# jzlianglu/pykaldi2

Measured on AMD Instinct MI355X. Metric: iRTF (hrs audio/hr) 3x512 BLSTM LF-MMI, LibriSpeech-shaped synthetic utterances, higher is better.
Workload: dtype f32 (GEMMs: bf16x3 split, f32 accumulate)

## Files before the change

include/pk2hip.h:

```cpp
#ifndef PK2HIP_H_
#define PK2HIP_H_

#include <stddef.h>
#include <stdint.h>

#ifdef __cplusplus
extern "C" {
#endif

typedef enum {
  PK2_OK = 0,
  PK2_ERR_INVALID = -1,
  PK2_ERR_HIP = -2,
  PK2_ERR_LIMIT = -3,
  PK2_ERR_IO = -4,
  PK2_ERR_NUMERIC = -5
} pk2_status;

const char* pk2_last_error(void);
int pk2_version(void);

typedef struct pk2_den_graph pk2_den_graph;

int pk2_den_graph_create(int32_t num_states, int32_t num_pdfs, int64_t num_arcs,
                         const int32_t* arc_src, const int32_t* arc_dst,
                         const int32_t* arc_pdf, const float* arc_prob,
                         int32_t start_state, pk2_den_graph** out);
int pk2_den_graph_from_openfst(const char* path, int32_t num_pdfs, pk2_den_graph** out);
int pk2_den_graph_destroy(pk2_den_graph* g);
int pk2_den_graph_info(const pk2_den_graph* g, int32_t* num_states, int32_t* num_pdfs,
                       int64_t* num_arcs);
int pk2_den_graph_initial_probs(const pk2_den_graph* g, float* host_out);

int32_t pk2_den_graph_path(const pk2_den_graph* g, int32_t num_seqs);
int32_t pk2_den_graph_persist_form(const pk2_den_graph* g, int32_t num_seqs);
int pk2_den_graph_plan(const pk2_den_graph* g, int32_t num_seqs, int32_t max_frames, int32_t out[8]);

typedef struct {
  const int32_t* arc_src;
  const int32_t* arc_dst;
  const int32_t* arc_pdf;
  const float* arc_weight;
  const int32_t* frame_off;
  const int32_t* state_off;
  const int32_t* final_state;
  const float* final_weight;
  const int32_t* final_off;
  int64_t total_arcs;
  int64_t max_seq_arcs;
} pk2_num_batch;

size_t pk2_chain_workspace_bytes(const pk2_den_graph* g, int32_t num_seqs, int32_t max_frames,
                                 int64_t num_total_states);

int pk2_chain_objf_and_deriv(const pk2_den_graph* g, const float* logits, int64_t seq_stride,
                             int64_t frame_stride, const int32_t* lengths, int32_t num_seqs,
                             const pk2_num_batch* num, float leaky_hmm_coefficient,
                             float xent_regularize, float l2_regularize, float weight,
                             float* grad, int64_t grad_seq_stride, int64_t grad_frame_stride,
                             float* out, void* workspace, size_t workspace_bytes, void* stream);

int pk2_chain_objf_and_deriv_op(const pk2_den_graph* g, const float* logits, int64_t seq_stride,
                                int64_t frame_stride, const int32_t* lengths, int32_t num_seqs,
                                const pk2_num_batch* num, float leaky_hmm_coefficient,
                                float xent_regularize, float l2_regularize, float weight,
                                float* grad, int64_t grad_seq_stride, int64_t grad_frame_stride,
                                float* out, void* workspace, size_t workspace_bytes, float grad_scale,
                                float* objf_sum, void* stream);

int pk2_chain_den_fwd_bwd(const pk2_den_graph* g, const float* logits, int64_t seq_stride,
                          int64_t frame_stride, const int32_t* lengths, int32_t num_seqs,
                          float leaky_hmm_coefficient, float* den_logprob, float* gamma,
                          int64_t gamma_seq_stride, int64_t gamma_frame_stride, void* workspace,
                          size_t workspace_bytes, void* stream);

int pk2_chain_debug_flags(const float* num_lp, const float* den_lp, const float* alpha_beta_product,
                          const int32_t* lengths, int32_t N, float weight, float* out, int32_t* flags, void* stream);

int pk2_chain_debug_num_route(int32_t out[4]);

int pk2_split_to_phones(const int32_t* tid_tstate, const int32_t* tid_phone, const uint8_t* tid_flags,
                        int32_t num_tids, const int32_t* alignment, int32_t T, int32_t* phones,
                        int32_t* durations, int32_t* num_phones, int32_t* ok);

typedef struct pk2_sup_model pk2_sup_model;
pk2_sup_model* pk2_sup_model_create(int32_t max_phone, const int32_t* phone2entry, int32_t num_entries,
                                    const int32_t* entry_state_off, const int32_t* state_fwd_class,
                                    const int32_t* state_loop_class, const int32_t* state_trans_off,
                                    const int32_t* trans_dst, int32_t num_tuples, const int32_t* tuples,
                                    int32_t context_width, int32_t central_position, int32_t num_nodes,
                                    const int32_t* node_kind, const int32_t* node_key, const int32_t* node_a,
                                    const int32_t* node_b, int32_t pool_size, const int32_t* pool);
void pk2_sup_model_destroy(pk2_sup_model* m);
int pk2_sup_model_pdf(const pk2_sup_model* m, const int32_t* window, int32_t pdf_class, int32_t* pdf);

typedef struct pk2_supervision pk2_supervision;
pk2_supervision* pk2_supervision_create(const pk2_sup_model* m, const int32_t* phones,
                                        const int32_t* durations, int32_t num_phones, int32_t subsampling,
                                        int32_t left_tolerance, int32_t right_tolerance);
void pk2_supervision_destroy(pk2_supervision* s);
void pk2_supervision_sizes(const pk2_supervision* s, int32_t* frames, int32_t* num_states, int32_t* num_arcs,
                           int32_t* num_final, int32_t* num_allowed);
int pk2_supervision_copy(const pk2_supervision* s, int32_t* arc_src, int32_t* arc_dst, int32_t* arc_pdf,
                         float* arc_weight, int32_t* frame_off, int32_t* state_time, int32_t* final_state,
                         float* final_weight, int32_t* allowed_off, int32_t* allowed_phones);

typedef struct pk2_lexicon pk2_lexicon;
pk2_lexicon* pk2_lexicon_create(int32_t num_states, int32_t start, int64_t num_arcs, const int32_t* src, const int32_t* dst,
                                const int32_t* ilabel, const int32_t* olabel, const float* weight, const float* final_cost,
                                const int32_t* disambig, int32_t num_disambig);
pk2_lexicon* pk2_lexicon_from_openfst(const char* path, const int32_t* disambig, int32_t num_disambig);
void pk2_lexicon_destroy(pk2_lexicon* lexicon);
typedef struct pk2_align_model pk2_align_model;
pk2_align_model* pk2_align_model_create(const pk2_sup_model* m, int32_t num_tuples, const int32_t* tuples, int32_t num_tids,
                                        const double* log_probs, double transition_scale, double self_loop_scale);
void pk2_align_model_destroy(pk2_align_model* model);
typedef struct pk2_align_graphs pk2_align_graphs;
pk2_align_graphs* pk2_align_compile(const pk2_align_model* model, const pk2_lexicon* lexicon, int32_t num_utts,
                                    const int32_t* word_off, const int32_t* words, const int32_t* frames);
void pk2_align_graphs_destroy(pk2_align_graphs* graphs);
int pk2_align_graphs_info(const pk2_align_graphs* graphs, int32_t utt, int32_t* status, int32_t* num_states, int32_t* num_arcs);
const char* pk2_align_graphs_error(const pk2_align_graphs* graphs, int32_t utt);
int pk2_align_graphs_copy(const pk2_align_graphs* graphs, int32_t utt, int32_t* in_off, int32_t* arc_src, int32_t* arc_tid,
                          int32_t* arc_pdf, float* arc_weight, float* final_cost);
int64_t pk2_align_graphs_packed_words(const pk2_align_graphs* graphs);
int pk2_align_graphs_pack(const pk2_align_graphs* graphs, int32_t* out);
size_t pk2_align_workspace_bytes(const pk2_align_graphs* graphs);
int pk2_align_use_lds(const pk2_align_graphs* graphs);
int pk2_align_viterbi(const pk2_align_graphs* graphs, const int32_t* packed_dev, const float* loglikes, int64_t seq_stride,
                      int64_t frame_stride, int32_t num_pdfs, int32_t Tmax, float acoustic_scale, float beam,
                      int32_t* alignment, float* costs, int32_t* status, void* workspace, size_t workspace_bytes,
                      void* stream);

size_t pk2_num_graph_workspace_bytes(const pk2_align_graphs* graphs);
int pk2_num_graph_use_lds(const pk2_align_graphs* graphs);
int pk2_num_graph_fwd_bwd(const pk2_align_graphs* graphs, const int32_t* packed_dev, const float* logits, int64_t seq_stride,
                          int64_t frame_stride, int32_t num_pdfs, int32_t Tmax, float scale, float* grad, int64_t grad_seq_stride,
                          int64_t grad_frame_stride, float* logprob, int32_t* status, void* workspace, size_t workspace_bytes,
                          void* stream);
size_t pk2_chain_graph_workspace_bytes(const pk2_den_graph* g, const pk2_align_graphs* graphs);
int pk2_chain_objf_and_deriv_graph(const pk2_den_graph* g, const float* logits, int64_t seq_stride, int64_t frame_stride,
                                   const pk2_align_graphs* graphs, const int32_t* packed_dev, float leaky_hmm_coefficient,
                                   float xent_regularize, float l2_regularize, float weight, float* grad,
                                   int64_t grad_seq_stride, int64_t grad_frame_stride, float* out, void* workspace,
                                   size_t workspace_bytes, void* stream);
int pk2_chain_objf_and_deriv_graph_op(const pk2_den_graph* g, const float* logits, int64_t seq_stride, int64_t frame_stride,
                                      const pk2_align_graphs* graphs, const int32_t* packed_dev, float leaky_hmm_coefficient,
                                      float xent_regularize, float l2_regularize, float weight, float* grad,
                                      int64_t grad_seq_stride, int64_t grad_frame_stride, float* out, void* workspace,
                                      size_t workspace_bytes, float grad_scale, float* objf_sum, void* stream);

int pk2_sim_apply_rir(const float* wav, int64_t n, const float* rir, int32_t k, int32_t delay, float* out,
                      void* stream);
int pk2_sim_apply_rir_dev(const float* wav, int64_t n, const float* rir, int32_t k, const int32_t* delay, float* out,
                          void* stream);
int pk2_sim_power(const float* x, int64_t n, double* stats, void* stream);
int pk2_sim_add_noise(float* mixed, int64_t n, const float* noise, int64_t m, int64_t start, float snr_db,
                      const double* sig_stats, const double* noise_stats, void* stream);
int pk2_sim_gain_norm(float* x, int64_t n, const double* stats, void* stream);

#define PK2_SIM_MAX_SEGS 16
typedef struct {
  const float* wav;
  const float* rir;
  float* out;
  float* early;
  const int32_t* delay_dev;
  int64_t n;
  int32_t k;
  int32_t delay;
} pk2_sim_rir_job;
int pk2_sim_apply_rir_mc(const pk2_sim_rir_job* jobs, int32_t njobs, int32_t channels, int32_t early_taps, void* stream);

typedef struct {
  float* x;
  int64_t count;
} pk2_sim_seg;
int pk2_sim_power_seg(const pk2_sim_seg* segs, int32_t nseg, double* stats, void* stream);
int pk2_sim_gain_norm_seg(const pk2_sim_seg* segs, int32_t nseg, const double* stats, double* gain, void* stream);

typedef struct {
  const float* sig;
  const float* sig2;
  float* pos;
  float* pos2;
  int64_t n;
  int64_t start;
  double spr_db;
} pk2_sim_mix_src;
int pk2_sim_mix(const pk2_sim_mix_src* srcs, int32_t nsrc, int32_t channels, int64_t T, const double* stats, float* mixed,
                double* scales, void* stream);
int pk2_sim_add_noise_mc(float* mixed, int64_t n, const float* noise, int64_t m, int32_t channels, int64_t start,
                         float snr_db, int32_t repeat, const double* sig_stats, const double* noise_stats, void* stream);

typedef struct pk2_resample_plan pk2_resample_plan;
#define PK2_RESAMPLE_MAX_TAPS 1024
int pk2_resample_plan_create(int32_t rate_in, int32_t rate_out, double cutoff_hz, int32_t num_zeros,
                             pk2_resample_plan** plan);
int pk2_resample_plan_destroy(pk2_resample_plan* plan);
int pk2_resample_plan_info(const pk2_resample_plan* plan, int32_t* iu, int32_t* ou, int32_t* max_taps, int32_t* tile,
                           int64_t* table_bytes);
int pk2_resample_plan_export(const pk2_resample_plan* plan, int32_t* first, int32_t* taps, float* weights);
int64_t pk2_resample_num_output(const pk2_resample_plan* plan, int64_t n_in);

#define PK2_RESAMPLE_MAX_JOBS 32
typedef struct {
  const pk2_resample_plan* plan;
  const float* in;
  int64_t n_in;
  float* out;
  int64_t n_out;
  float gain;
} pk2_resample_job;
int pk2_resample_batch(const pk2_resample_job* jobs, int32_t njobs, void* stream);
#define PK2_RESAMPLE_PATH_NONE 0
#define PK2_RESAMPLE_PATH_LDS 1
#define PK2_RESAMPLE_PATH_MEM 2
int pk2_resample_last_path(int32_t* path);

int pk2_iso_spectra(const double* tau, const double* g, const float* draws, uint64_t seed, int32_t channels, int32_t points,
                    int32_t bins, float* X, void* stream);
int pk2_iso_gauss(uint64_t seed, int32_t points, int32_t bins, float* out, void* stream);

int pk2_irfft_pow2_f32(const float* X, int32_t rows, int32_t n, float* out, void* stream);

int64_t pk2_stft_num_frames(int64_t n, int32_t frame_len, int32_t frame_shift);
int pk2_stft_f32(const float* const* rows, int32_t R, int64_t n, int32_t fft_size, int32_t frame_len, int32_t frame_shift,
                 const float* window, const float* dither, int32_t use_seed, uint64_t seed, float* out, void* stream);
int pk2_istft_f32(const float* X, int32_t R, int32_t N, int32_t fft_size, int32_t frame_len, int32_t frame_shift,
                  const float* window, float* work, float* out, void* stream);
int pk2_mask_power(const float* spec, int64_t count, float* power, void* stream);
size_t pk2_mask_count_workspace_bytes(int32_t S);
int pk2_mask_count_threshold(const float* power, int32_t S, int64_t m, double energy_threshold, void* work, size_t work_bytes,
                             float* out, void* stream);
int pk2_mask_ibm(const float* clean, const float* distorted, int32_t S, int32_t N, int32_t F, float snr_factor, int32_t soft,
                 const float* thr, const float* vad, float* mask, void* stream);

#define PK2_RIR_F64 16
#define PK2_RIR_I64 12
int32_t pk2_rirgen_segment_samples(void);
int pk2_rirgen(const double* item_f64, const int64_t* item_i64, const double* pos, const int32_t* wg, int32_t nwg,
               const int32_t* row_item, int32_t nrows, int64_t total, void* acc, float* out, int32_t* delay,
               void* stream);

typedef struct pk2_fbank pk2_fbank;
int pk2_fbank_create(const float* mel_80x257, pk2_fbank** out);
int pk2_fbank_destroy(pk2_fbank* fb);
int32_t pk2_fbank_num_frames(int64_t num_samples);
int pk2_fbank_compute(const pk2_fbank* fb, const float* wav, const int64_t* wav_off,
                      int32_t num_utts, float* feats, const int64_t* feat_row_off,
                      int32_t apply_cmn, void* stream);
int pk2_pad_roll_subsample(const float* feats, const int64_t* feat_row_off, int32_t num_utts,
                           int32_t max_t, int32_t shift, int32_t subsample, float* x,
                           int32_t out_t, int32_t time_major, void* stream);

int pk2_mvn_apply(const float* x, const float* mean, const float* stdv, int64_t rows, int32_t dim,
                  float* y, void* stream);

#define PK2_SPEC_MAX_FREQ_MASKS 4
#define PK2_SPEC_MAX_TIME_MASKS 16
#define PK2_SPEC_PLAN_STRIDE (2 + 2 * PK2_SPEC_MAX_FREQ_MASKS + 2 * PK2_SPEC_MAX_TIME_MASKS)
int pk2_spec_augment(const float* in, float* out, const int64_t* row_off , int32_t n,
                     int64_t total_rows, const int32_t* plan , int32_t has_warp,
                     float fill, void* stream);

#define PK2_BF_MAX_CHANNELS 8
#define PK2_BF_MAX_MASKS 4
#define PK2_BF_MAX_UTTS 32
#define PK2_BF_FRAMES_PER_PART 32
#define PK2_BF_REF_SNR (-1)
size_t pk2_bf_workspace_bytes(const int32_t* frames, int32_t B, int32_t C, int32_t F, int32_t K, int32_t complement);
int pk2_bf_cov(const float* const* spec, const float* const* masks, const int32_t* frames, int32_t B, int32_t C, int32_t F,
               int32_t K, int32_t complement, void* work, size_t work_bytes, float* phi, void* stream);
int pk2_bf_mvdr_weights(const float* const* phi_s, const float* const* phi_n, int32_t B, int32_t C, int32_t F, int32_t ref,
                        double diag_load, void* work, size_t work_bytes, float* w, int32_t* ref_index, int32_t* nonfinite,
                        void* stream);
int pk2_bf_apply(const float* const* spec, const float* const* w, const int32_t* frames, int32_t B, int32_t C, int32_t F,
                 float* const* out, void* stream);

#define PK2_WPE_MAX_CHANNELS 8
#define PK2_WPE_MAX_ORDER 80
#define PK2_WPE_MAX_DELAY 8
#define PK2_WPE_MAX_ITERS 8
#define PK2_WPE_MAX_UTTS 32
#define PK2_WPE_FRAMES_PER_PART 1024
size_t pk2_wpe_workspace_bytes(const int32_t* frames, int32_t B, int32_t C, int32_t F, int32_t taps, int32_t delay);
int pk2_wpe_power(const float* const* spec, const int32_t* frames, int32_t B, int32_t C, int32_t F, float* const* power,
                  void* stream);
int pk2_wpe_corr(const float* const* spec, const float* const* weight, const int32_t* frames, int32_t B, int32_t C, int32_t F,
                 int32_t taps, int32_t delay, void* work, size_t work_bytes, float* R, float* P, void* stream);
int pk2_wpe_solve(const float* R, const float* P, int32_t B, int32_t C, int32_t F, int32_t taps, double diag_load, void* work,
                  size_t work_bytes, float* G, int32_t* nonfinite, void* stream);
int pk2_wpe_filter(const float* const* spec, const float* G, const int32_t* frames, int32_t B, int32_t C, int32_t F,
                   int32_t taps, int32_t delay, float* const* out, float* const* power_out, void* stream);
int pk2_wpe(const float* const* spec, const int32_t* frames, int32_t B, int32_t C, int32_t F, int32_t taps, int32_t delay,
            int32_t iters, double diag_load, void* work, size_t work_bytes, float* const* out, int32_t* nonfinite,
            void* stream);

#define PK2_CGMM_MAX_ITERS 32
size_t pk2_cgmm_workspace_bytes(const int32_t* frames, int32_t B, int32_t C, int32_t F, int32_t K);
int pk2_cgmm_init(const float* const* spec, const float* const* init, const float* const* activity, const int32_t* frames,
                  int32_t B, int32_t C, int32_t F, int32_t K, void* work, size_t work_bytes, float* R, float* log_alpha,
                  void* stream);
int pk2_cgmm_factor(const float* R, const float* log_alpha, int32_t B, int32_t C, int32_t F, int32_t K, double diag_load,
                    float* linv, float* bias, int32_t* bad, int32_t* nonfinite, void* stream);
int pk2_cgmm_posteriors(const float* const* spec, const float* const* activity, const int32_t* frames, int32_t B, int32_t C,
                        int32_t F, int32_t K, const float* linv, const float* bias, const int32_t* bad, void* work,
                        size_t work_bytes, float* const* lam, float* const* phi, double* ll, void* stream);
int pk2_cgmm_update(const float* const* spec, const float* const* lam, const float* const* phi, const float* const* activity,
                    const int32_t* frames, int32_t B, int32_t C, int32_t F, int32_t K, void* work, size_t work_bytes, float* R,
                    float* log_alpha, void* stream);
int pk2_cgmm(const float* const* spec, const float* const* init, const float* const* activity, const int32_t* frames, int32_t B,
             int32_t C, int32_t F, int32_t K, int32_t iters, double diag_load, int32_t purity, void* work, size_t work_bytes,
             float* const* masks, float* R, float* log_alpha, double* ll, int32_t* nonfinite, void* stream);

#define PK2_PERM_ALIGN_MAX_REFINE 8
size_t pk2_perm_align_workspace_bytes(const int32_t* frames, int32_t B, int32_t F, int32_t K);
int pk2_perm_align(const float* const* masks, const float* cov, const float* log_alpha, const int32_t* frames, int32_t B,
                   int32_t C, int32_t F, int32_t K, int32_t refine, int32_t noise_last, void* work, size_t work_bytes,
                   float* const* out_masks, float* out_cov, float* out_log_alpha, int32_t* perm, float* margin, void* stream);

int pk2_softmax_ce_fwd_bwd(const float* logits, int64_t row_stride, const int64_t* targets,
                           int64_t ignore_index, int64_t rows, int32_t num_classes,
                           float* loss_sum, int32_t* count, float* grad, int64_t grad_row_stride,
                           float* logprob_out , void* stream);
int pk2_softmax_ce_fwd_bwd_mean(const float* logits, int64_t row_stride, const int64_t* targets,
                                int64_t ignore_index, int64_t rows, int32_t num_classes,
                                float* loss_sum, int32_t* count, float* grad, int64_t grad_row_stride, void* stream);
int pk2_scale_inplace_ratio(float* data, int64_t n, const float* num_dev, const float* den_dev, void* stream);
int pk2_scale_by_count(float* data, int64_t n, float numerator, const int32_t* count_den,
                       void* stream);
int pk2_scale_by_scalars(const float* in, float* out, int64_t n, const float* mul_dev, const int32_t* count_den_dev,
                         void* stream);

int pk2_gemm_f32(int32_t transa, int32_t transb, int32_t M, int32_t N, int32_t K, float alpha,
                 const float* A, int64_t lda, const float* B, int64_t ldb, float beta, float* C,
                 int64_t ldc, const float* bias, void* stream);
int pk2_gemm_f32_act(int32_t transa, int32_t transb, int32_t M, int32_t N, int32_t K, float alpha,
                     const float* A, int64_t lda, const float* B, int64_t ldb, float beta, float* C,
                     int64_t ldc, const float* bias, int32_t act, const float* gate, int64_t ldg, void* stream);
int pk2_gemm_f32_seg(int32_t transa, int32_t transb, int32_t M, int32_t N, int32_t K, int32_t nseg, float alpha,
                     const float* A, int64_t lda, int64_t segA, const float* B, int64_t ldb, int64_t segB, float beta,
                     float* C, int64_t ldc, const float* bias, int32_t act, const float* gate, int64_t ldg,
                     void* stream);
int pk2_gemm_f32_batched(int32_t transa, int32_t transb, int32_t M, int32_t N, int32_t K, float alpha,
                         const float* A, int64_t lda, int64_t strideA0, int64_t strideA1, const float* B,
                         int64_t ldb, int64_t strideB0, int64_t strideB1, float beta, float* C, int64_t ldc,
                         int64_t strideC0, int64_t strideC1, int32_t n0, int32_t n1, void* stream);
int pk2_gemm_set_arith(int32_t arith);
int pk2_gemm_get_arith(void);
int pk2_gemm_f32_tn_colsum(int32_t M, int32_t N, int32_t K, float alpha, const float* A, int64_t lda, const float* B,
                           int64_t ldb, float beta, float* C, int64_t ldc, float* colsum, void* stream);
int pk2_colsum_f32(const float* A, int64_t lda, int32_t M, int32_t N, float beta, float* out,
                   void* stream);

size_t pk2_lstm_fwd_workspace_floats(int32_t B, int32_t H, int32_t num_dirs);
int pk2_lstm_layer_fwd(const float* gx, const float* whh, const float* bhh, int32_t B, int32_t T,
                       int32_t H, int32_t num_dirs, float* y, float* gates, float* cells,
                       void* workspace, void* stream);
int pk2_lstm_layer_fwd_xproj(const float* gx, const float* whh, const float* bhh, int32_t B, int32_t T,
                             int32_t H, int32_t num_dirs, float* y, float* gates, float* cells, void* workspace,
                             const float* inp, int32_t in_size, const float* w_ih, const float* b_ih,
                             int32_t* gx_done, void* stream);
int pk2_lstm_persist_status(uint32_t* abort_flag);
#define PK2_LSTM_PATH_NONE 0
#define PK2_LSTM_PATH_SEQ 1
#define PK2_LSTM_PATH_BIG 2
#define PK2_LSTM_PATH_BIG_AG 3
#define PK2_LSTM_PATH_STEP_SMALL 4
#define PK2_LSTM_PATH_STEP_BIG 5
int pk2_lstm_last_path(int32_t* fwd, int32_t* bwd);
size_t pk2_lstm_bwd_scratch_floats(int32_t B, int32_t H, int32_t num_dirs);
int pk2_lstm_layer_bwd(const float* dy, const float* whh, const float* gates, const float* cells,
                       int32_t B, int32_t T, int32_t H, int32_t num_dirs, float* dgx,
                       float* scratch, void* stream);
int pk2_lstm_layer_bwd_bias(const float* dy, const float* whh, const float* gates, const float* cells,
                            int32_t B, int32_t T, int32_t H, int32_t num_dirs, float* dgx, float* scratch,
                            float* dbias_ih, float* dbias_hh, int32_t* bias_done, void* stream);
size_t pk2_lstm_bwd_wgrad_workspace_floats(int32_t B, int32_t H, int32_t num_dirs);
int pk2_lstm_layer_bwd_wgrad(const float* dy, const float* whh, const float* gates, const float* cells, const float* y,
                             int32_t B, int32_t T, int32_t H, int32_t num_dirs, float* dgx, float* scratch,
                             float* dbias_ih, float* dbias_hh, float* dwhh, float* wgrad_ws, int32_t* bias_done,
                             int32_t* whh_done, void* stream);

int pk2_layernorm_fwd(const float* x, const float* res, const float* gamma, const float* beta, int64_t rows,
                      int32_t C, float eps, float* sum_out, float* y, float* mean, float* rstd, void* stream);
int pk2_layernorm_bwd(const float* dy, const float* s, const float* mean, const float* rstd,
                      const float* gamma, int64_t rows, int32_t C, float* ds, float* dgamma, float* dbeta,
                      void* stream);
int pk2_softmax_mask_fwd(float* scores, const float* src_mask, const uint8_t* key_padding, int32_t B, int32_t H,
                         int32_t T, void* stream);
int pk2_softmax_bwd(const float* P, float* dP, int32_t BH, int32_t T, void* stream);

int pk2_attention_fwd(const float* qkv, int32_t T, int32_t B, int32_t H, int32_t head_dim, float scale,
                      const float* src_mask, const uint8_t* key_padding, float dropout_p, uint64_t seed, float* ctx,
                      float* lse, void* stream);
int pk2_attention_bwd(const float* qkv, const float* ctx, const float* dctx, const float* lse, int32_t T, int32_t B,
                      int32_t H, int32_t head_dim, float scale, const float* src_mask, const uint8_t* key_padding,
                      float dropout_p, uint64_t seed, float* dqkv, float* dsum, void* stream);
int pk2_attention_bwd_part(int32_t parts, const float* qkv, const float* ctx, const float* dctx, const float* lse, int32_t T,
                           int32_t B, int32_t H, int32_t head_dim, float scale, const float* src_mask,
                           const uint8_t* key_padding, float dropout_p, uint64_t seed, float* dqkv, float* dsum, void* stream);
int pk2_relu_fwd(float* x, int64_t n, void* stream);
int pk2_relu_bwd(const float* y, float* dy, int64_t n, void* stream);
int pk2_add_inplace(float* a, const float* b, int64_t n, void* stream);

int pk2_dropout_f32(const float* x, float* y, int64_t n, float p, uint64_t seed, void* stream);

int pk2_grad_norm(const float* grad, int64_t n, float* norm_out, void* workspace,
                  size_t workspace_bytes, void* stream);
size_t pk2_grad_norm_workspace_bytes(int64_t n);
int pk2_adam_step(float* param, const float* grad, float* exp_avg, float* exp_avg_sq,
                  float* max_exp_avg_sq , int64_t n, float lr, float beta1,
                  float beta2, float eps, float weight_decay, int64_t step, float max_norm,
                  const float* norm, float grad_scale, void* stream);
int pk2_sgd_step(float* param, const float* grad, float* momentum_buf ,
                 int64_t n, float lr, float momentum, float weight_decay, int32_t first_step,
                 float max_norm, const float* norm, float grad_scale, void* stream);

int pk2_persist_guard_status(uint32_t* raised);
int pk2_persist_guard_clear(void);
int pk2_persist_guard_raise(void* stream);
int pk2_persist_guard_export(float* slot, void* stream);
int pk2_persist_guard_import(const float* slot, uint32_t stamp, void* stream);
int pk2_persist_guard_verdict(uint32_t stamp, uint32_t* ready, uint32_t* raised);

typedef struct pk2_decode_graph pk2_decode_graph;

int pk2_decode_graph_create(int32_t num_states, int32_t start_state, int64_t num_arcs,
                            const int32_t* arc_src, const int32_t* arc_dst, const int32_t* arc_ilabel,
                            const float* arc_weight, const float* final_cost, pk2_decode_graph** out);
int pk2_decode_graph_from_openfst(const char* path, pk2_decode_graph** out);
int pk2_decode_graph_create_words(int32_t num_states, int32_t start_state, int64_t num_arcs,
                                  const int32_t* arc_src, const int32_t* arc_dst, const int32_t* arc_ilabel,
                                  const int32_t* arc_olabel, const float* arc_weight, const float* final_cost,
                                  pk2_decode_graph** out);
int pk2_decode_graph_link_words(const pk2_decode_graph* g, int64_t num_links, const int32_t* src_state,
                                const int32_t* dst_state, const int32_t* tid, const float* graph_cost,
                                int32_t* word_out);
int pk2_decode_graph_destroy(pk2_decode_graph* g);
int pk2_decode_graph_info(const pk2_decode_graph* g, int32_t* num_states, int64_t* num_arcs,
                          int32_t* max_ilabel);

typedef struct {
  float beam;
  float lattice_beam;
  float beam_delta;
  float acoustic_scale;
  int32_t max_active;
  int32_t min_active;
  int32_t tokens_per_frame;
  int32_t links_per_frame;
} pk2_decoder_opts;

typedef struct pk2_lattice_batch pk2_lattice_batch;
int pk2_lattice_batch_create(const pk2_decode_graph* g, const int32_t* lengths_host, int32_t num_seq,
                             const pk2_decoder_opts* opts, pk2_lattice_batch** out);
size_t pk2_lattice_batch_bytes(const pk2_lattice_batch* b);
int pk2_lattice_batch_destroy(pk2_lattice_batch* b);

int pk2_lattice_decode(pk2_lattice_batch* b, const float* loglikes, int64_t seq_stride,
                       int64_t frame_stride, int32_t num_pdfs, const int32_t* tid2pdf, int32_t num_tids,
                       void* workspace, void* stream);
int pk2_lattice_persist_status(int32_t* state, uint32_t* abort_flag);
int pk2_lattice_summary(const pk2_lattice_batch* b, const void* workspace, int32_t* status,
                        int32_t* num_tokens, int32_t* num_links, float* best_cost, void* stream);
int pk2_lattice_fb_rerun(const pk2_lattice_batch* b, void* workspace, int32_t* rerun, void* stream);
int pk2_lattice_mmi(const pk2_lattice_batch* b, void* workspace, const int32_t* ref_tids,
                    int64_t ref_stride, const int32_t* tid2pdf, double lm_scale, double acoustic_scale,
                    int32_t drop_frames, float* post, int64_t post_seq_stride,
                    int64_t post_frame_stride, double* lat_like, void* stream);
int pk2_lattice_mpe(const pk2_lattice_batch* b, void* workspace, const int32_t* ref_tids,
                    int64_t ref_stride, const int32_t* tid2pdf, const int32_t* tid2phone,
                    const uint8_t* phone_is_silence, int32_t criterion, int32_t one_silence_class,
                    double lm_scale, double acoustic_scale, float* post, int64_t post_seq_stride,
                    int64_t post_frame_stride, double* score, void* stream);
size_t pk2_lattice_nbest_bytes(const pk2_lattice_batch* b, int32_t num_paths, int64_t total_tokens, int64_t total_links,
                               int32_t distinct, int32_t label_cap);
int pk2_lattice_nbest(const pk2_lattice_batch* b, void* workspace, void* scratch, int64_t total_tokens,
                      int64_t total_links, int32_t num_paths, int32_t distinct, int32_t label_mode,
                      const int32_t* tid2label, int32_t num_tids, double lm_scale, double acoustic_scale,
                      int32_t label_cap, int32_t* num_hyp, int32_t* hyp_path, float* path_cost, int32_t* path_nlab,
                      int32_t* path_labels, int32_t* path_tids, void* stream);
int pk2_lattice_mwe(const pk2_lattice_batch* b, void* workspace, void* scratch, int64_t total_tokens,
                    int64_t total_links, int32_t num_paths, int32_t distinct, int32_t label_mode,
                    const int32_t* tid2label, int32_t num_tids, double lm_scale, double acoustic_scale,
                    int32_t label_cap, int32_t equal_weight, const int32_t* sup, int64_t sup_stride,
                    const int32_t* sup_len, const int32_t* tid2pdf, int32_t num_pdfs, float* grad,
                    int64_t grad_seq_stride, int64_t grad_frame_stride, double* loss, void* stream);
int pk2_lattice_rescore(const pk2_lattice_batch* b, void* workspace, const float* loglikes, int64_t seq_stride,
                        int64_t frame_stride, int32_t num_pdfs, const int32_t* tid2pdf, int32_t num_tids,
                        float old_acoustic_scale, void* stream);
int pk2_lattice_posteriors(const pk2_lattice_batch* b, void* workspace, const int32_t* tid2pdf, double lm_scale,
                           double acoustic_scale, float post_sign, float* post, int64_t post_seq_stride,
                           int64_t post_frame_stride, double* lat_like, void* stream);
int pk2_lattice_ts(const pk2_lattice_batch* b, void* workspace, const float* loglikes_S, int64_t seq_stride,
                   int64_t frame_stride, int32_t num_pdfs, const int32_t* tid2pdf, int32_t num_tids,
                   float old_acoustic_scale, double lm_scale, double acoustic_scale, float* grad,
                   int64_t grad_seq_stride, int64_t grad_frame_stride, double* loss, double* like_T, double* like_S,
                   void* stream);
int pk2_lattice_export(const pk2_lattice_batch* b, const void* workspace, int32_t n, int32_t* num_tokens,
                       int32_t* num_links, int32_t* tok_frame, int32_t* tok_state, float* tok_cost,
                       float* tok_final, int32_t* link_src, int32_t* link_dst, int32_t* link_tid,
                       float* link_graph, float* link_ac, void* stream);

typedef struct pk2_det_lattice pk2_det_lattice;
int pk2_lattice_determinize(int32_t num_states, int32_t start, int64_t num_arcs, const int32_t* src, const int32_t* dst,
                            const int32_t* word, const int32_t* tid, const float* graph, const float* acoustic,
                            const float* final_cost, double beam, int64_t max_states, pk2_det_lattice** out);
int pk2_det_lattice_sizes(const pk2_det_lattice* h, int32_t* num_states, int32_t* start, int64_t* num_arcs,
                          int64_t* arc_tids, int64_t* final_tids);
int pk2_det_lattice_export(const pk2_det_lattice* h, int32_t* src, int32_t* dst, int32_t* word, float* graph,
                           float* acoustic, int64_t* tid_off, int32_t* tids, float* final_graph, float* final_acoustic,
                           int64_t* final_tid_off, int32_t* final_tids);
void pk2_det_lattice_destroy(pk2_det_lattice* h);

typedef struct pk2_comm pk2_comm;
int32_t pk2_comm_unique_id_bytes(void);
int pk2_comm_unique_id(void* id_out);
int pk2_comm_init(int32_t rank, int32_t world, const void* unique_id, pk2_comm** out);
int pk2_allreduce_bucket(pk2_comm* comm, float* buf, int64_t count, void* stream);
int pk2_allreduce_guarded(pk2_comm* comm, float* buf, int64_t count, float* guard_slot, void* stream);
int pk2_comm_info(const pk2_comm* comm, int32_t* rank, int32_t* world, char* lib_path, int32_t lib_path_bytes);
int pk2_comm_destroy(pk2_comm* comm);

int pk2_stream_create_cu_mask(int32_t cus_per_xcd, void** stream_out);
int pk2_stream_destroy(void* stream);
int pk2_debug_where(int32_t* out, int32_t blocks, void* stream);
int pk2_debug_peer_reduce(float* dst, const float* src, int64_t n, int32_t blocks, int32_t passes, void* stream);

#ifdef __cplusplus
}
#endif
#endif
```

pykaldi2_amd/_lib.py:

```python
import ctypes as C
import os

import torch

_HERE = os.path.dirname(os.path.abspath(__file__))
LIB_PATH = os.environ.get("PK2_LIB") or os.path.join(_HERE, "libpk2hip.so")


class Pk2Error(RuntimeError):
    pass


class NumBatch(C.Structure):
    _fields_ = [("arc_src", C.c_void_p), ("arc_dst", C.c_void_p), ("arc_pdf", C.c_void_p),
                ("arc_weight", C.c_void_p), ("frame_off", C.c_void_p), ("state_off", C.c_void_p),
                ("final_state", C.c_void_p), ("final_weight", C.c_void_p), ("final_off", C.c_void_p),
                ("total_arcs", C.c_int64), ("max_seq_arcs", C.c_int64)]


class DecoderOpts(C.Structure):
    _fields_ = [("beam", C.c_float), ("lattice_beam", C.c_float), ("beam_delta", C.c_float),
                ("acoustic_scale", C.c_float), ("max_active", C.c_int32), ("min_active", C.c_int32),
                ("tokens_per_frame", C.c_int32), ("links_per_frame", C.c_int32)]


class SimRirJob(C.Structure):
    _fields_ = [("wav", C.c_void_p), ("rir", C.c_void_p), ("out", C.c_void_p), ("early", C.c_void_p),
                ("delay_dev", C.c_void_p), ("n", C.c_int64), ("k", C.c_int32), ("delay", C.c_int32)]


class SimSeg(C.Structure):
    _fields_ = [("x", C.c_void_p), ("count", C.c_int64)]


class SimMixSrc(C.Structure):
    _fields_ = [("sig", C.c_void_p), ("sig2", C.c_void_p), ("pos", C.c_void_p), ("pos2", C.c_void_p),
                ("n", C.c_int64), ("start", C.c_int64), ("spr_db", C.c_double)]


class ResampleJob(C.Structure):
    _fields_ = [("plan", C.c_void_p), ("inp", C.c_void_p), ("n_in", C.c_int64), ("out", C.c_void_p), ("n_out", C.c_int64),
                ("gain", C.c_float)]


SIM_MAX_SEGS = 16
RESAMPLE_MAX_JOBS = 32
SPEC_MAX_FREQ_MASKS = 4
SPEC_MAX_TIME_MASKS = 16
SPEC_PLAN_STRIDE = 2 + 2 * SPEC_MAX_FREQ_MASKS + 2 * SPEC_MAX_TIME_MASKS
BF_MAX_CHANNELS = 8
BF_MAX_MASKS = 4
BF_FRAMES_PER_PART = 32
BF_REF_SNR = -1
CGMM_MAX_ITERS = 32
PERM_ALIGN_MAX_REFINE = 8
WPE_MAX_CHANNELS = 8
WPE_MAX_ORDER = 80
WPE_MAX_DELAY = 8
WPE_MAX_ITERS = 8
WPE_FRAMES_PER_PART = 1024

_vp, _i32, _i64, _f32, _sz = C.c_void_p, C.c_int32, C.c_int64, C.c_float, C.c_size_t

SIGNATURES = {
    "pk2_last_error": (C.c_char_p, []),
    "pk2_version": (C.c_int, []),
    "pk2_den_graph_create": (C.c_int, [_i32, _i32, _i64, _vp, _vp, _vp, _vp, _i32, C.POINTER(_vp)]),
    "pk2_den_graph_from_openfst": (C.c_int, [C.c_char_p, _i32, C.POINTER(_vp)]),
    "pk2_den_graph_destroy": (C.c_int, [_vp]),
    "pk2_den_graph_info": (C.c_int, [_vp, C.POINTER(_i32), C.POINTER(_i32), C.POINTER(_i64)]),
    "pk2_den_graph_initial_probs": (C.c_int, [_vp, _vp]),
    "pk2_den_graph_arcs_per_lane": (_i32, []),
    "pk2_den_graph_path": (_i32, [_vp, _i32]),
    "pk2_den_graph_persist_form": (_i32, [_vp, _i32]),
    "pk2_den_graph_plan": (C.c_int, [_vp, _i32, _i32, _vp]),
    "pk2_den_graph_debug_ordering": (C.c_int, [_vp, C.c_int, C.POINTER(_i64), C.POINTER(_i32), _vp, _vp,
                                               _vp, _vp, _vp, _vp]),
    "pk2_den_graph_debug_virtual": (C.c_int, [_vp, C.c_int, C.POINTER(_i32), _vp, _vp, _vp, _vp, _vp,
                                              C.POINTER(_i64), _vp, _vp, _vp, C.POINTER(_i32), _vp, _vp]),
    "pk2_den_graph_debug_persist2": (C.c_int, [_vp, C.c_int] + [_vp] * 18),
    "pk2_den_graph_debug_persist2_table": (C.c_int, [_vp, C.c_int, _vp, _vp, _vp, _vp]),
    "pk2_chain_workspace_bytes": (_sz, [_vp, _i32, _i32, _i64]),
    "pk2_chain_objf_and_deriv": (C.c_int, [_vp, _vp, _i64, _i64, _vp, _i32, C.POINTER(NumBatch), _f32,
                                           _f32, _f32, _f32, _vp, _i64, _i64, _vp, _vp, _sz, _vp]),
    "pk2_chain_objf_and_deriv_op": (C.c_int, [_vp, _vp, _i64, _i64, _vp, _i32, C.POINTER(NumBatch), _f32,
                                              _f32, _f32, _f32, _vp, _i64, _i64, _vp, _vp, _sz, _f32, _vp, _vp]),
    "pk2_chain_den_fwd_bwd": (C.c_int, [_vp, _vp, _i64, _i64, _vp, _i32, _f32, _vp, _vp, _i64, _i64,
                                        _vp, _sz, _vp]),
    "pk2_chain_debug_flags": (C.c_int, [_vp, _vp, _vp, _vp, _i32, _f32, _vp, _vp, _vp]),
    "pk2_chain_debug_num_route": (C.c_int, [_vp]),
    "pk2_split_to_phones": (C.c_int, [_vp, _vp, _vp, _i32, _vp, _i32, _vp, _vp, C.POINTER(_i32), C.POINTER(_i32)]),
    "pk2_sup_model_create": (_vp, [_i32, _vp, _i32, _vp, _vp, _vp, _vp, _vp, _i32, _vp, _i32, _i32, _i32, _vp, _vp,
                                   _vp, _vp, _i32, _vp]),
    "pk2_sup_model_destroy": (None, [_vp]),
    "pk2_sup_model_pdf": (C.c_int, [_vp, _vp, _i32, C.POINTER(_i32)]),
    "pk2_supervision_create": (_vp, [_vp, _vp, _vp, _i32, _i32, _i32, _i32]),
    "pk2_supervision_destroy": (None, [_vp]),
    "pk2_supervision_sizes": (None, [_vp, C.POINTER(_i32), C.POINTER(_i32), C.POINTER(_i32), C.POINTER(_i32),
                                     C.POINTER(_i32)]),
    "pk2_supervision_copy": (C.c_int, [_vp, _vp, _vp, _vp, _vp, _vp, _vp, _vp, _vp, _vp, _vp]),
    "pk2_lexicon_create": (_vp, [_i32, _i32, _i64, _vp, _vp, _vp, _vp, _vp, _vp, _vp, _i32]),
    "pk2_lexicon_from_openfst": (_vp, [C.c_char_p, _vp, _i32]),
    "pk2_lexicon_destroy": (None, [_vp]),
    "pk2_align_model_create": (_vp, [_vp, _i32, _vp, _i32, _vp, C.c_double, C.c_double]),
    "pk2_align_model_destroy": (None, [_vp]),
    "pk2_align_compile": (_vp, [_vp, _vp, _i32, _vp, _vp, _vp]),
    "pk2_align_graphs_destroy": (None, [_vp]),
    "pk2_align_graphs_info": (C.c_int, [_vp, _i32, C.POINTER(_i32), C.POINTER(_i32), C.POINTER(_i32)]),
    "pk2_align_graphs_error": (C.c_char_p, [_vp, _i32]),
    "pk2_align_graphs_copy": (C.c_int, [_vp, _i32, _vp, _vp, _vp, _vp, _vp, _vp]),
    "pk2_align_graphs_packed_words": (_i64, [_vp]),
    "pk2_align_graphs_pack": (C.c_int, [_vp, _vp]),
    "pk2_align_workspace_bytes": (_sz, [_vp]),
    "pk2_align_use_lds": (C.c_int, [_vp]),
    "pk2_align_viterbi": (C.c_int, [_vp, _vp, _vp, _i64, _i64, _i32, _i32, _f32, _f32, _vp, _vp, _vp, _vp, _sz, _vp]),
    "pk2_num_graph_workspace_bytes": (_sz, [_vp]),
    "pk2_num_graph_use_lds": (C.c_int, [_vp]),
    "pk2_num_graph_fwd_bwd": (C.c_int, [_vp, _vp, _vp, _i64, _i64, _i32, _i32, _f32, _vp, _i64, _i64, _vp, _vp, _vp, _sz, _vp]),
    "pk2_chain_graph_workspace_bytes": (_sz, [_vp, _vp]),
    "pk2_chain_objf_and_deriv_graph": (C.c_int, [_vp, _vp, _i64, _i64, _vp, _vp, _f32, _f32, _f32, _f32, _vp, _i64, _i64, _vp,
                                                 _vp, _sz, _vp]),
    "pk2_chain_objf_and_deriv_graph_op": (C.c_int, [_vp, _vp, _i64, _i64, _vp, _vp, _f32, _f32, _f32, _f32, _vp, _i64, _i64,
                                                    _vp, _vp, _sz, _f32, _vp, _vp]),
    "pk2_decode_graph_create": (C.c_int, [_i32, _i32, _i64, _vp, _vp, _vp, _vp, _vp, C.POINTER(_vp)]),
    "pk2_decode_graph_create_words": (C.c_int, [_i32, _i32, _i64, _vp, _vp, _vp, _vp, _vp, _vp, C.POINTER(_vp)]),
    "pk2_decode_graph_link_words": (C.c_int, [_vp, _i64, _vp, _vp, _vp, _vp, _vp]),
    "pk2_decode_graph_from_openfst": (C.c_int, [C.c_char_p, C.POINTER(_vp)]),
    "pk2_decode_graph_destroy": (C.c_int, [_vp]),
    "pk2_decode_graph_info": (C.c_int, [_vp, C.POINTER(_i32), C.POINTER(_i64), C.POINTER(_i32)]),
    "pk2_lattice_batch_create": (C.c_int, [_vp, _vp, _i32, C.POINTER(DecoderOpts), C.POINTER(_vp)]),
    "pk2_lattice_batch_bytes": (_sz, [_vp]),
    "pk2_lattice_batch_destroy": (C.c_int, [_vp]),
    "pk2_lattice_decode": (C.c_int, [_vp, _vp, _i64, _i64, _i32, _vp, _i32, _vp, _vp]),
    "pk2_lattice_summary": (C.c_int, [_vp, _vp, _vp, _vp, _vp, _vp, _vp]),
    "pk2_lattice_persist_status": (C.c_int, [C.POINTER(C.c_int32), C.POINTER(C.c_uint32)]),
    "pk2_lattice_mmi": (C.c_int, [_vp, _vp, _vp, _i64, _vp, C.c_double, C.c_double, _i32, _vp, _i64, _i64, _vp, _vp]),
    "pk2_lattice_mpe": (C.c_int, [_vp, _vp, _vp, _i64, _vp, _vp, _vp, _i32, _i32, C.c_double, C.c_double, _vp, _i64, _i64,
                                  _vp, _vp]),
    "pk2_lattice_nbest_bytes": (_sz, [_vp, _i32, _i64, _i64, _i32, _i32]),
    "pk2_lattice_nbest": (C.c_int, [_vp, _vp, _vp, _i64, _i64, _i32, _i32, _i32, _vp, _i32, C.c_double, C.c_double, _i32,
                                    _vp, _vp, _vp, _vp, _vp, _vp, _vp]),
    "pk2_lattice_mwe": (C.c_int, [_vp, _vp, _vp, _i64, _i64, _i32, _i32, _i32, _vp, _i32, C.c_double, C.c_double, _i32, _i32,
                                  _vp, _i64, _vp, _vp, _i32, _vp, _i64, _i64, _vp, _vp]),
    "pk2_lattice_rescore": (C.c_int, [_vp, _vp, _vp, _i64, _i64, _i32, _vp, _i32, _f32, _vp]),
    "pk2_lattice_fb_rerun": (C.c_int, [_vp, _vp, _vp, _vp]),
    "pk2_lattice_posteriors": (C.c_int, [_vp, _vp, _vp, C.c_double, C.c_double, _f32, _vp, _i64, _i64, _vp, _vp]),
    "pk2_lattice_ts": (C.c_int, [_vp, _vp, _vp, _i64, _i64, _i32, _vp, _i32, _f32, C.c_double, C.c_double, _vp, _i64, _i64,
                                 _vp, _vp, _vp, _vp]),
    "pk2_lattice_export": (C.c_int, [_vp, _vp, _i32, C.POINTER(_i32), C.POINTER(_i32), _vp, _vp, _vp, _vp, _vp,
                                     _vp, _vp, _vp, _vp, _vp]),
    "pk2_comm_unique_id_bytes": (_i32, []),
    "pk2_comm_unique_id": (C.c_int, [_vp]),
    "pk2_comm_init": (C.c_int, [_i32, _i32, _vp, C.POINTER(_vp)]),
    "pk2_allreduce_bucket": (C.c_int, [_vp, _vp, _i64, _vp]),
    "pk2_allreduce_guarded": (C.c_int, [_vp, _vp, _i64, _vp, _vp]),
    "pk2_comm_info": (C.c_int, [_vp, C.POINTER(_i32), C.POINTER(_i32), C.c_char_p, _i32]),
    "pk2_comm_destroy": (C.c_int, [_vp]),
    "pk2_sim_apply_rir": (C.c_int, [_vp, _i64, _vp, _i32, _i32, _vp, _vp]),
    "pk2_sim_apply_rir_dev": (C.c_int, [_vp, _i64, _vp, _i32, _vp, _vp, _vp]),
    "pk2_sim_power": (C.c_int, [_vp, _i64, _vp, _vp]),
    "pk2_rirgen_segment_samples": (_i32, []),
    "pk2_rirgen": (C.c_int, [_vp, _vp, _vp, _vp, _i32, _vp, _i32, _i64, _vp, _vp, _vp, _vp]),
    "pk2_sim_add_noise": (C.c_int, [_vp, _i64, _vp, _i64, _i64, _f32, _vp, _vp, _vp]),
    "pk2_sim_gain_norm": (C.c_int, [_vp, _i64, _vp, _vp]),
    "pk2_sim_apply_rir_mc": (C.c_int, [C.POINTER(SimRirJob), _i32, _i32, _i32, _vp]),
    "pk2_sim_power_seg": (C.c_int, [C.POINTER(SimSeg), _i32, _vp, _vp]),
    "pk2_sim_gain_norm_seg": (C.c_int, [C.POINTER(SimSeg), _i32, _vp, _vp, _vp]),
    "pk2_sim_mix": (C.c_int, [C.POINTER(SimMixSrc), _i32, _i32, _i64, _vp, _vp, _vp, _vp]),
    "pk2_sim_add_noise_mc": (C.c_int, [_vp, _i64, _vp, _i64, _i32, _i64, _f32, _i32, _vp, _vp, _vp]),
    "pk2_resample_plan_create": (C.c_int, [_i32, _i32, C.c_double, _i32, C.POINTER(_vp)]),
    "pk2_resample_plan_destroy": (C.c_int, [_vp]),
    "pk2_resample_plan_info": (C.c_int, [_vp, C.POINTER(_i32), C.POINTER(_i32), C.POINTER(_i32), C.POINTER(_i32),
                                         C.POINTER(_i64)]),
    "pk2_resample_plan_export": (C.c_int, [_vp, _vp, _vp, _vp]),
    "pk2_resample_num_output": (_i64, [_vp, _i64]),
    "pk2_resample_batch": (C.c_int, [C.POINTER(ResampleJob), _i32, _vp]),
    "pk2_resample_last_path": (C.c_int, [C.POINTER(_i32)]),
    "pk2_iso_spectra": (C.c_int, [_vp, _vp, _vp, C.c_uint64, _i32, _i32, _i32, _vp, _vp]),
    "pk2_iso_gauss": (C.c_int, [C.c_uint64, _i32, _i32, _vp, _vp]),
    "pk2_irfft_pow2_f32": (C.c_int, [_vp, _i32, _i32, _vp, _vp]),
    "pk2_stft_num_frames": (_i64, [_i64, _i32, _i32]),
    "pk2_stft_f32": (C.c_int, [C.POINTER(_vp), _i32, _i64, _i32, _i32, _i32, _vp, _vp, _i32, C.c_uint64, _vp, _vp]),
    "pk2_istft_f32": (C.c_int, [_vp, _i32, _i32, _i32, _i32, _i32, _vp, _vp, _vp, _vp]),
    "pk2_mask_power": (C.c_int, [_vp, _i64, _vp, _vp]),
    "pk2_mask_count_workspace_bytes": (_sz, [_i32]),
    "pk2_mask_count_threshold": (C.c_int, [_vp, _i32, _i64, C.c_double, _vp, _sz, _vp, _vp]),
    "pk2_mask_ibm": (C.c_int, [_vp, _vp, _i32, _i32, _i32, _f32, _i32, _vp, _vp, _vp, _vp]),
    "pk2_fbank_create": (C.c_int, [_vp, C.POINTER(_vp)]),
    "pk2_fbank_destroy": (C.c_int, [_vp]),
    "pk2_fbank_num_frames": (_i32, [_i64]),
    "pk2_fbank_compute": (C.c_int, [_vp, _vp, _vp, _i32, _vp, _vp, _i32, _vp]),
    "pk2_pad_roll_subsample": (C.c_int, [_vp, _vp, _i32, _i32, _i32, _i32, _vp, _i32, _i32, _vp]),
    "pk2_mvn_apply": (C.c_int, [_vp, _vp, _vp, _i64, _i32, _vp, _vp]),
    "pk2_spec_augment": (C.c_int, [_vp, _vp, _vp, _i32, _i64, _vp, _i32, _f32, _vp]),
    "pk2_bf_workspace_bytes": (_sz, [_vp, _i32, _i32, _i32, _i32, _i32]),
    "pk2_bf_cov": (C.c_int, [C.POINTER(_vp), C.POINTER(_vp), C.POINTER(_i32), _i32, _i32, _i32, _i32, _i32, _vp, _sz, _vp, _vp]),
    "pk2_bf_mvdr_weights": (C.c_int, [C.POINTER(_vp), C.POINTER(_vp), _i32, _i32, _i32, _i32, C.c_double, _vp, _sz, _vp, _vp,
                                      _vp, _vp]),
    "pk2_bf_apply": (C.c_int, [C.POINTER(_vp), C.POINTER(_vp), C.POINTER(_i32), _i32, _i32, _i32, C.POINTER(_vp), _vp]),
    "pk2_wpe_workspace_bytes": (_sz, [_vp, _i32, _i32, _i32, _i32, _i32]),
    "pk2_wpe_power": (C.c_int, [C.POINTER(_vp), C.POINTER(_i32), _i32, _i32, _i32, C.POINTER(_vp), _vp]),
    "pk2_wpe_corr": (C.c_int, [C.POINTER(_vp), C.POINTER(_vp), C.POINTER(_i32), _i32, _i32, _i32, _i32, _i32, _vp, _sz, _vp, _vp,
                               _vp]),
    "pk2_wpe_solve": (C.c_int, [_vp, _vp, _i32, _i32, _i32, _i32, C.c_double, _vp, _sz, _vp, _vp, _vp]),
    "pk2_wpe_filter": (C.c_int, [C.POINTER(_vp), _vp, C.POINTER(_i32), _i32, _i32, _i32, _i32, _i32, C.POINTER(_vp),
                                 C.POINTER(_vp), _vp]),
    "pk2_wpe": (C.c_int, [C.POINTER(_vp), C.POINTER(_i32), _i32, _i32, _i32, _i32, _i32, _i32, C.c_double, _vp, _sz,
                          C.POINTER(_vp), _vp, _vp]),
    "pk2_cgmm_workspace_bytes": (_sz, [_vp, _i32, _i32, _i32, _i32]),
    "pk2_cgmm_init": (C.c_int, [C.POINTER(_vp), C.POINTER(_vp), C.POINTER(_vp), C.POINTER(_i32), _i32, _i32, _i32, _i32, _vp, _sz,
                                _vp, _vp, _vp]),
    "pk2_cgmm_factor": (C.c_int, [_vp, _vp, _i32, _i32, _i32, _i32, C.c_double, _vp, _vp, _vp, _vp, _vp]),
    "pk2_cgmm_posteriors": (C.c_int, [C.POINTER(_vp), C.POINTER(_vp), C.POINTER(_i32), _i32, _i32, _i32, _i32, _vp, _vp, _vp, _vp,
                                      _sz, C.POINTER(_vp), C.POINTER(_vp), _vp, _vp]),
    "pk2_cgmm_update": (C.c_int, [C.POINTER(_vp), C.POINTER(_vp), C.POINTER(_vp), C.POINTER(_vp), C.POINTER(_i32), _i32, _i32,
                                  _i32, _i32, _vp, _sz, _vp, _vp, _vp]),
    "pk2_cgmm": (C.c_int, [C.POINTER(_vp), C.POINTER(_vp), C.POINTER(_vp), C.POINTER(_i32), _i32, _i32, _i32, _i32, _i32,
                           C.c_double, _i32, _vp, _sz, C.POINTER(_vp), _vp, _vp, _vp, _vp, _vp]),
    "pk2_perm_align_workspace_bytes": (_sz, [_vp, _i32, _i32, _i32]),
    "pk2_perm_align": (C.c_int, [C.POINTER(_vp), _vp, _vp, C.POINTER(_i32), _i32, _i32, _i32, _i32, _i32, _i32, _vp, _sz,
                                 C.POINTER(_vp), _vp, _vp, _vp, _vp, _vp]),
    "pk2_softmax_ce_fwd_bwd": (C.c_int, [_vp, _i64, _vp, _i64, _i64, _i32, _vp, _vp, _vp, _i64, _vp, _vp]),
    "pk2_softmax_ce_fwd_bwd_mean": (C.c_int, [_vp, _i64, _vp, _i64, _i64, _i32, _vp, _vp, _vp, _i64, _vp]),
    "pk2_scale_inplace_ratio": (C.c_int, [_vp, _i64, _vp, _vp, _vp]),
    "pk2_scale_by_count": (C.c_int, [_vp, _i64, _f32, _vp, _vp]),
    "pk2_scale_by_scalars": (C.c_int, [_vp, _vp, _i64, _vp, _vp, _vp]),
    "pk2_gemm_f32": (C.c_int, [_i32, _i32, _i32, _i32, _i32, _f32, _vp, _i64, _vp, _i64, _f32, _vp, _i64,
                               _vp, _vp]),
    "pk2_gemm_f32_act": (C.c_int, [_i32, _i32, _i32, _i32, _i32, _f32, _vp, _i64, _vp, _i64, _f32, _vp, _i64, _vp, _i32, _vp, _i64,
                                   _vp]),
    "pk2_gemm_f32_seg": (C.c_int, [_i32, _i32, _i32, _i32, _i32, _i32, _f32, _vp, _i64, _i64, _vp, _i64, _i64, _f32, _vp, _i64, _vp,
                                   _i32, _vp, _i64, _vp]),
    "pk2_gemm_f32_batched": (C.c_int, [_i32, _i32, _i32, _i32, _i32, _f32, _vp, _i64, _i64, _i64, _vp, _i64, _i64, _i64,
                                       _f32, _vp, _i64, _i64, _i64, _i32, _i32, _vp]),
    "pk2_gemm_f32_tn_colsum": (C.c_int, [_i32, _i32, _i32, _f32, _vp, _i64, _vp, _i64, _f32, _vp, _i64, _vp, _vp]),
    "pk2_gemm_set_arith": (C.c_int, [_i32]),
    "pk2_gemm_get_arith": (C.c_int, []),
    "pk2_layernorm_fwd": (C.c_int, [_vp, _vp, _vp, _vp, _i64, _i32, _f32, _vp, _vp, _vp, _vp, _vp]),
    "pk2_layernorm_bwd": (C.c_int, [_vp, _vp, _vp, _vp, _vp, _i64, _i32, _vp, _vp, _vp, _vp]),
    "pk2_softmax_mask_fwd": (C.c_int, [_vp, _vp, _vp, _i32, _i32, _i32, _vp]),
    "pk2_softmax_bwd": (C.c_int, [_vp, _vp, _i32, _i32, _vp]),
    "pk2_attention_fwd": (C.c_int, [_vp, _i32, _i32, _i32, _i32, _f32, _vp, _vp, _f32, C.c_uint64, _vp, _vp, _vp]),
    "pk2_attention_bwd": (C.c_int, [_vp, _vp, _vp, _vp, _i32, _i32, _i32, _i32, _f32, _vp, _vp, _f32, C.c_uint64, _vp,
                                    _vp, _vp]),
    "pk2_attention_bwd_part": (C.c_int, [_i32, _vp, _vp, _vp, _vp, _i32, _i32, _i32, _i32, _f32, _vp, _vp, _f32, C.c_uint64,
                                         _vp, _vp, _vp]),
    "pk2_relu_fwd": (C.c_int, [_vp, _i64, _vp]),
    "pk2_relu_bwd": (C.c_int, [_vp, _vp, _i64, _vp]),
    "pk2_add_inplace": (C.c_int, [_vp, _vp, _i64, _vp]),
    "pk2_colsum_f32": (C.c_int, [_vp, _i64, _i32, _i32, _f32, _vp, _vp]),
    "pk2_lstm_fwd_workspace_floats": (_sz, [_i32, _i32, _i32]),
    "pk2_lstm_layer_fwd": (C.c_int, [_vp, _vp, _vp, _i32, _i32, _i32, _i32, _vp, _vp, _vp, _vp, _vp]),
    "pk2_lstm_layer_fwd_xproj": (C.c_int, [_vp, _vp, _vp, _i32, _i32, _i32, _i32, _vp, _vp, _vp, _vp, _vp, _i32, _vp, _vp,
                                           C.POINTER(_i32), _vp]),
    "pk2_lstm_persist_status": (C.c_int, [C.POINTER(C.c_uint32)]),
    "pk2_lstm_last_path": (C.c_int, [C.POINTER(_i32), C.POINTER(_i32)]),
    "pk2_lattice_determinize": (C.c_int, [_i32, _i32, _i64, _vp, _vp, _vp, _vp, _vp, _vp, _vp, C.c_double, _i64, C.POINTER(_vp)]),
    "pk2_det_lattice_sizes": (C.c_int, [_vp, C.POINTER(_i32), C.POINTER(_i32), C.POINTER(_i64), C.POINTER(_i64), C.POINTER(_i64)]),
    "pk2_det_lattice_export": (C.c_int, [_vp] * 12),
    "pk2_det_lattice_destroy": (None, [_vp]),
    "pk2_persist_guard_status": (C.c_int, [C.POINTER(C.c_uint32)]),
    "pk2_persist_guard_clear": (C.c_int, []),
    "pk2_persist_guard_raise": (C.c_int, [_vp]),
    "pk2_persist_guard_export": (C.c_int, [_vp, _vp]),
    "pk2_persist_guard_import": (C.c_int, [_vp, C.c_uint32, _vp]),
    "pk2_persist_guard_verdict": (C.c_int, [C.c_uint32, C.POINTER(C.c_uint32), C.POINTER(C.c_uint32)]),
    "pk2_lstm_bwd_scratch_floats": (_sz, [_i32, _i32, _i32]),
    "pk2_lstm_layer_bwd_bias": (C.c_int, [_vp, _vp, _vp, _vp, _i32, _i32, _i32, _i32, _vp, _vp, _vp, _vp, C.POINTER(_i32), _vp]),
    "pk2_lstm_layer_bwd": (C.c_int, [_vp, _vp, _vp, _vp, _i32, _i32, _i32, _i32, _vp, _vp, _vp]),
    "pk2_lstm_bwd_wgrad_workspace_floats": (_sz, [_i32, _i32, _i32]),
    "pk2_lstm_layer_bwd_wgrad": (C.c_int, [_vp, _vp, _vp, _vp, _vp, _i32, _i32, _i32, _i32, _vp, _vp, _vp, _vp, _vp, _vp,
                                           C.POINTER(_i32), C.POINTER(_i32), _vp]),
    "pk2_dropout_f32": (C.c_int, [_vp, _vp, _i64, _f32, C.c_uint64, _vp]),
    "pk2_grad_norm": (C.c_int, [_vp, _i64, _vp, _vp, _sz, _vp]),
    "pk2_grad_norm_workspace_bytes": (_sz, [_i64]),
    "pk2_adam_step": (C.c_int, [_vp, _vp, _vp, _vp, _vp, _i64, _f32, _f32, _f32, _f32, _f32, _i64, _f32,
                                _vp, _f32, _vp]),
    "pk2_sgd_step": (C.c_int, [_vp, _vp, _vp, _i64, _f32, _f32, _f32, _i32, _f32, _vp, _f32, _vp]),
    "pk2_stream_create_cu_mask": (C.c_int, [_i32, C.POINTER(_vp)]),
    "pk2_stream_destroy": (C.c_int, [_vp]),
    "pk2_debug_where": (C.c_int, [_vp, _i32, _vp]),
    "pk2_debug_peer_reduce": (C.c_int, [_vp, _vp, _i64, _i32, _i32, _vp]),
}

_lib = None


def lib():
    global _lib
    if _lib is None:
        if not os.path.exists(LIB_PATH):
            raise Pk2Error("%s is missing: run `python -c 'import __graft_entry__ as g; g.build()'` "
                           "(hipcc --offload-arch=gfx950).  There is no CPU fallback." % LIB_PATH)
        handle = C.CDLL(LIB_PATH)
        for name, (res, args) in SIGNATURES.items():
            fn = getattr(handle, name)
            fn.restype = res
            fn.argtypes = args
        _lib = handle
    return _lib


def h2d(host, device):
    import numpy as np
    t = torch.from_numpy(host) if isinstance(host, np.ndarray) else host
    if torch.device(device).type != "cuda" or t.is_cuda or t.numel() == 0:
        return t.to(device)
    return t.contiguous().pin_memory().to(device, non_blocking=True)


def check(status):
    if status != 0:
        msg = lib().pk2_last_error()
        raise Pk2Error("libpk2hip status %d: %s" % (status, msg.decode() if msg else ""))


def persist_guard_raised():
    flag = C.c_uint32(0)
    check(lib().pk2_persist_guard_status(C.byref(flag)))
    return flag.value != 0


def check_persist_guard(where, raised=None):
    if persist_guard_raised() if raised is None else raised:
        raise Pk2Error("%s: a persistent kernel (one-launch LSTM recurrence / denominator / lattice decoder) timed out on "
                       "this device; its output was poisoned with NaN and the optimiser kernels have been leaving the "
                       "weights untouched since.  Typical causes: the GPU is shared with another process, or fewer than "
                       "256 CUs are available to the launch.  PK2_LSTM_SEQ=0 PK2_LSTM_BIG_PERSIST=0 PK2_DEN_PERSIST=0 "
                       "PK2_LAT_DECODER=frames select the launch-per-step kernels." % where)


def ptr(t):
    if t is None:
        return None
    if isinstance(t, torch.Tensor):
        return C.c_void_p(t.data_ptr())
    return C.c_void_p(t.ctypes.data)


def stream_ptr(device=None):
    return C.c_void_p(torch.cuda.current_stream(device).cuda_stream)


def require_gpu():
    if not torch.cuda.is_available():
        raise Pk2Error("pykaldi2_amd needs an MI355X (torch.cuda.is_available() is False); "
                       "there is no CPU fallback")
```

pykaldi2_amd/csrc/gemm_bf16x3.h:

```cpp
#pragma once
#include "gemm_tile.h"

namespace pk2 {

typedef __bf16 bf16x8_t __attribute__((ext_vector_type(8)));
typedef unsigned int u32x4_t __attribute__((ext_vector_type(4)));

template <int TILES> struct GeoX {
  static constexpr int BMN = 64 * TILES;
  static constexpr int BK = TILES == 2 ? 16 : 32;
  static constexpr int NKG = BK / 8;
  static constexpr int NQ = BMN / 4;
  static constexpr int SW = NQ + 4;
  template <bool KC> static constexpr int sp() { return KC ? BMN + 4 : NQ + 3 * SW; }
  template <bool KC> static constexpr int slots() { return 3 * NKG * sp<KC>(); }
  template <bool KC> __device__ static __forceinline__ int slot(int row) { return KC ? row : (row >> 2) + SW * (row & 3); }
};

__device__ __forceinline__ unsigned pk_bf16(float a, float b) {
  typedef __bf16 bf16x2_t __attribute__((ext_vector_type(2)));
  typedef float f32x2_t __attribute__((ext_vector_type(2)));
  f32x2_t v = {a, b};
  bf16x2_t r = __builtin_convertvector(v, bf16x2_t);
  return __builtin_bit_cast(unsigned, r);
}
__device__ __forceinline__ void split_pair(float x0, float x1, unsigned& h, unsigned& m, unsigned& l) {
  h = pk_bf16(x0, x1);
#ifdef PK2_X3_DBG_NOSPLIT
  m = h; l = h; return;
#endif
  const float r0 = x0 - __uint_as_float(h << 16), r1 = x1 - __uint_as_float(h & 0xffff0000u);
  m = pk_bf16(r0, r1);
  const float s0 = r0 - __uint_as_float(m << 16), s1 = r1 - __uint_as_float(m & 0xffff0000u);
  l = pk_bf16(s0, s1);
}

template <bool KC, int TILES> struct PieceMap {
  int row[2], k[2];
  int kg, d;
  __device__ __forceinline__ PieceMap() {
    const int t = threadIdx.x;
    if (KC) {
      if (TILES == 2) { row[0] = t >> 2; row[1] = (t >> 2) + 64; k[0] = k[1] = (t & 3) * 4; }
      else            { row[0] = row[1] = t >> 2; k[0] = (t & 3) * 4; k[1] = k[0] + 16; }
      kg = d = 0;
    } else {
      const int q = (t & 7) + 8 * ((t >> 5) & (TILES == 2 ? 3 : 1));
      d = (t >> 3) & 3;
      kg = TILES == 2 ? (t >> 7) : (t >> 6);
      row[0] = row[1] = 4 * q;
      k[0] = 8 * kg + 2 * d;
      k[1] = k[0] + 1;
    }
  }
};

template <bool KC, int TILES>
__device__ __forceinline__ void xslab_pointers(const PieceMap<KC, TILES>& pm, const float* __restrict__ base, int64_t ld, int r0,
                                               int k0, int R, const float* (&ptr)[2], int64_t* step) {
#pragma unroll
  for (int h = 0; h < 2; ++h) {
    if (KC) ptr[h] = base + (int64_t)min(r0 + pm.row[h], R - 1) * ld + k0 + pm.k[h];
    else    ptr[h] = base + (int64_t)(k0 + pm.k[h]) * ld + min(r0 + pm.row[h], R - 4);
  }
  *step = KC ? (int64_t)GeoX<TILES>::BK : (int64_t)GeoX<TILES>::BK * ld;
}

template <bool KC, int TILES>
__device__ __forceinline__ void xload_general(const PieceMap<KC, TILES>& pm, const float* __restrict__ base, int64_t ld, int r0,
                                              int k0, int R, int K, bool vec, float4 (&reg)[2]) {
#pragma unroll
  for (int h = 0; h < 2; ++h) {
    const int gr = r0 + pm.row[h], gk = k0 + pm.k[h];
    float4 v = make_float4(0.f, 0.f, 0.f, 0.f);
    if (KC) {
      if (gr < R) {
        const float* p = base + (int64_t)gr * ld + gk;
        if (vec && gk + 3 < K) v = *reinterpret_cast<const float4*>(p);
        else {
          if (gk + 0 < K) v.x = p[0];
          if (gk + 1 < K) v.y = p[1];
          if (gk + 2 < K) v.z = p[2];
          if (gk + 3 < K) v.w = p[3];
        }
      }
    } else {
      if (gk < K) {
        const float* p = base + (int64_t)gk * ld + gr;
        if (vec && gr + 3 < R) v = *reinterpret_cast<const float4*>(p);
        else {
          if (gr + 0 < R) v.x = p[0];
          if (gr + 1 < R) v.y = p[1];
          if (gr + 2 < R) v.z = p[2];
          if (gr + 3 < R) v.w = p[3];
        }
      }
    }
    reg[h] = v;
  }
}

template <bool KC, int TILES, bool CS = false>
__device__ __forceinline__ void xstore(const PieceMap<KC, TILES>& pm, u32x4_t* __restrict__ tile, const float4 (&reg)[2],
                                       float* cs = nullptr, float csw = 0.f) {
  typedef GeoX<TILES> G;
  constexpr int SP = G::template sp<KC>(), PL = G::NKG * SP;
  if (KC) {
#pragma unroll
    for (int h = 0; h < 2; ++h) {
      unsigned h0, m0, l0, h1, m1, l1;
      split_pair(reg[h].x, reg[h].y, h0, m0, l0);
      split_pair(reg[h].z, reg[h].w, h1, m1, l1);
      const int kq = pm.k[h] >> 2;
      uint2* p = reinterpret_cast<uint2*>(tile + (kq >> 1) * SP + pm.row[h]) + (kq & 1);
      p[0] = make_uint2(h0, h1);
      p[2 * PL] = make_uint2(m0, m1);
      p[4 * PL] = make_uint2(l0, l1);
    }
  } else {
    const float a[4] = {reg[0].x, reg[0].y, reg[0].z, reg[0].w};
    const float b[4] = {reg[1].x, reg[1].y, reg[1].z, reg[1].w};
    unsigned* p = reinterpret_cast<unsigned*>(tile + pm.kg * SP + (pm.row[0] >> 2)) + pm.d;
#pragma unroll
    for (int i = 0; i < 4; ++i) {
      unsigned hh, mm, ll;
      split_pair(a[i], b[i], hh, mm, ll);
      p[4 * (G::SW * i)] = hh;
      p[4 * (G::SW * i + PL)] = mm;
      p[4 * (G::SW * i + 2 * PL)] = ll;
      if (CS) cs[i] = fmaf(csw, a[i] + b[i], cs[i]);
    }
  }
}

template <bool KCA, bool KCB, int TILES>
__device__ __forceinline__ void tile_mainloop_bf16x3(const float* __restrict__ A, int64_t lda, const float* __restrict__ B, int64_t ldb,
                                                     int m0, int n0, int kbeg, int K, int M, int N, bool vecA, bool vecB,
                                                     u32x4_t (*As)[GeoX<TILES>::template slots<KCA>()],
                                                     u32x4_t (*Bs)[GeoX<TILES>::template slots<KCB>()],
                                                     f32x16 (&acc)[TILES][TILES], float* __restrict__ colsum = nullptr,
                                                     bool zero_acc = true) {
  typedef GeoX<TILES> G;
  constexpr int BM = G::BMN, BN = G::BMN, XBK = G::BK, NKG = G::NKG;
  constexpr int SPA = G::template sp<KCA>(), SPB = G::template sp<KCB>();
  const int lane = threadIdx.x & 63, w = threadIdx.x >> 6;
  const int wm = (w >> 1) * 32 * TILES, wn = (w & 1) * 32 * TILES;
  if (zero_acc) {
#pragma unroll
    for (int i = 0; i < TILES; ++i)
#pragma unroll
      for (int j = 0; j < TILES; ++j)
#pragma unroll
        for (int r = 0; r < 16; ++r) acc[i][j][r] = 0.f;
  }
  const int kq = lane >> 5, li = lane & 31;
#ifndef PK2_GEMMX_DEPTH
#define PK2_GEMMX_DEPTH 2
#endif
  constexpr int DEPTH = PK2_GEMMX_DEPTH;
  static_assert(DEPTH % 2 == 0, "an even number of register stages (the LDS buffer is the stage's parity)");
  float4 ra[DEPTH][2], rb[DEPTH][2];
  const PieceMap<KCA, TILES> pma;
  const PieceMap<KCB, TILES> pmb;
  float cs[4] = {0.f, 0.f, 0.f, 0.f};
  const bool do_cs = !KCA && colsum != nullptr;
  auto store_a = [&](u32x4_t* tile, const float4 (&reg)[2], bool real = true) {
    if constexpr (!KCA) { if (do_cs) { xstore<KCA, TILES, true>(pma, tile, reg, cs, real ? 1.f : 0.f); return; } }
    xstore<KCA, TILES>(pma, tile, reg);
  };
  const int nk = (K - kbeg + XBK - 1) / XBK;
  const bool interior = vecA && vecB && (m0 + BM <= M || KCA || ((M & 3) == 0 && M >= 4)) &&
                        (n0 + BN <= N || KCB || ((N & 3) == 0 && N >= 4));
  const float* pa[2]; const float* pb[2];
  int64_t stepA = 0, stepB = 0;
  xslab_pointers<KCA, TILES>(pma, A, lda, m0, kbeg, M, pa, &stepA);
  xslab_pointers<KCB, TILES>(pmb, B, ldb, n0, kbeg, N, pb, &stepB);
  int sa[TILES], sb[TILES];
#pragma unroll
  for (int i = 0; i < TILES; ++i) sa[i] = kq * SPA + G::template slot<KCA>(wm + i * 32 + li);
#pragma unroll
  for (int j = 0; j < TILES; ++j) sb[j] = kq * SPB + G::template slot<KCB>(wn + j * 32 + li);
  auto multiply = [&](auto C_) {
    constexpr int cur = decltype(C_)::value;
#pragma unroll
    for (int s = 0; s < NKG / 2; ++s) {
      bf16x8_t a[3][TILES], b[3][TILES];
#pragma unroll
      for (int p = 0; p < 3; ++p) {
#pragma unroll
        for (int i = 0; i < TILES; ++i) a[p][i] = __builtin_bit_cast(bf16x8_t, As[cur][(p * NKG + 2 * s) * SPA + sa[i]]);
#pragma unroll
        for (int j = 0; j < TILES; ++j) b[p][j] = __builtin_bit_cast(bf16x8_t, Bs[cur][(p * NKG + 2 * s) * SPB + sb[j]]);
      }
#define PK2_X3(PA, PB)                                                                                   \
  _Pragma("unroll") for (int i = 0; i < TILES; ++i) _Pragma("unroll") for (int j = 0; j < TILES; ++j)    \
      acc[i][j] = __builtin_amdgcn_mfma_f32_32x32x16_bf16(a[PA][i], b[PB][j], acc[i][j], 0, 0, 0)
#ifdef PK2_X3_DBG_ONEMFMA
      PK2_X3(0, 0);
      asm volatile("" :: "v"(a[1][0]), "v"(a[2][0]), "v"(b[1][0]), "v"(b[2][0]));
#else
      PK2_X3(2, 0); PK2_X3(0, 2); PK2_X3(1, 1); PK2_X3(1, 0); PK2_X3(0, 1); PK2_X3(0, 0);
#endif
#undef PK2_X3
    }
  };
  auto pipeline = [&](int n, auto fetch) {
    if (n <= 0) return;
#pragma unroll
    for (int i = 0; i < DEPTH; ++i) fetch(min(i, n - 1), ra[i], rb[i]);
    store_a(As[0], ra[0]);
    xstore<KCB, TILES>(pmb, Bs[0], rb[0]);
    lds_barrier();
    fetch(min(DEPTH, n - 1), ra[0], rb[0]);
#ifndef PK2_GEMMX_PIN
#define PK2_GEMMX_PIN 1
#endif
    auto pin = [] { if (PK2_GEMMX_PIN) __builtin_amdgcn_sched_barrier(0); };
    auto slab_step = [&](int kt, auto P) {
      constexpr int st = decltype(P)::value, cur = st & 1, nxt = 1 - cur, sn = (st + 1) % DEPTH;
      multiply(std::integral_constant<int, cur>());
      if (kt + 1 < n) {
        store_a(As[nxt], ra[sn]);
        xstore<KCB, TILES>(pmb, Bs[nxt], rb[sn]);
      }
      lds_barrier();
      if (kt + 1 + DEPTH < n) fetch(kt + 1 + DEPTH, ra[sn], rb[sn]);
    };
    auto steady_step = [&](int kt, auto P) {
      constexpr int st = decltype(P)::value, cur = st & 1, nxt = 1 - cur, sn = (st + 1) % DEPTH;
      multiply(std::integral_constant<int, cur>());
      store_a(As[nxt], ra[sn], kt + 1 < n);
      xstore<KCB, TILES>(pmb, Bs[nxt], rb[sn]);
      lds_barrier();
      fetch(min(kt + 1 + DEPTH, n - 1), ra[sn], rb[sn]);
      pin();
    };
    int kt = 0;
    for (; kt + DEPTH <= n; kt += DEPTH)
      static_for<0, DEPTH>([&](auto S) { steady_step(kt + decltype(S)::value, S); });
    if (kt < n)
      static_for<0, DEPTH>([&](auto S) { if (kt + decltype(S)::value < n) slab_step(kt + decltype(S)::value, S); });
  };
  if (interior) {
    const int nk_fast = (K - kbeg) / XBK;
    pipeline(nk_fast, [&](int ks, float4 (&xa)[2], float4 (&xb)[2]) {
#ifdef PK2_X3_DBG_NOLOAD
      ks = 0;
#endif
#pragma unroll
      for (int h = 0; h < 2; ++h) xa[h] = *reinterpret_cast<const float4*>(pa[h] + ks * stepA);
#pragma unroll
      for (int h = 0; h < 2; ++h) xb[h] = *reinterpret_cast<const float4*>(pb[h] + ks * stepB);
    });
    if (nk > nk_fast) {
      xload_general<KCA, TILES>(pma, A, lda, m0, kbeg + nk_fast * XBK, M, K, vecA, ra[0]);
      xload_general<KCB, TILES>(pmb, B, ldb, n0, kbeg + nk_fast * XBK, N, K, vecB, rb[0]);
      store_a(As[0], ra[0]);
      xstore<KCB, TILES>(pmb, Bs[0], rb[0]);
      lds_barrier();
      multiply(std::integral_constant<int, 0>());
      lds_barrier();
    }
  } else {
    pipeline(nk, [&](int ks, float4 (&xa)[2], float4 (&xb)[2]) {
      xload_general<KCA, TILES>(pma, A, lda, m0, kbeg + ks * XBK, M, K, vecA, xa);
      xload_general<KCB, TILES>(pmb, B, ldb, n0, kbeg + ks * XBK, N, K, vecB, xb);
    });
  }
  if constexpr (!KCA) {
    if (do_cs) {
      float* red = reinterpret_cast<float*>(&As[0][0]);
      for (int r = threadIdx.x; r < BM; r += kGemmThreads) red[r] = 0.f;
      lds_barrier();
#pragma unroll
      for (int i = 0; i < 4; ++i) atomicAdd(&red[pma.row[0] + i], cs[i]);
      lds_barrier();
      for (int r = threadIdx.x; r < BM; r += kGemmThreads)
        if (m0 + r < M) atomicAdd(colsum + m0 + r, red[r]);
      lds_barrier();
    }
  }
}



}
```

pykaldi2_amd/csrc/gemm_f32.hip:

```cpp
#include <algorithm>
#include <cstdlib>
#include <type_traits>

#include "common.h"
#include "gemm_tile.h"
#include "gemm_bf16x3.h"

namespace pk2 {

struct GemmBatch { int n1; int64_t sA0, sA1, sB0, sB1, sC0, sC1; int ksplit, klen; float* colsum = nullptr;
                   int act = 0; const float* gate = nullptr; int64_t ldg = 0;
                   int nseg = 1; int64_t segA = 0, segB = 0; };

#ifndef PK2_GEMMX_WAVES
#define PK2_GEMMX_WAVES 2
#endif
template <int TILES>
__device__ __forceinline__ void gemm_store(const f32x16 (&acc)[TILES][TILES], int M, int N, float alpha, float beta, float* __restrict__ C,
                                           int64_t ldc, const float* __restrict__ bias, int m0, int n0, int wm, int wn, bool atomic,
                                           int act = 0, const float* __restrict__ gate = nullptr, int64_t ldg = 0) {
  const int lane = threadIdx.x & 63;
  const int col_l = lane & 31, row_h = 4 * (lane >> 5);
#pragma unroll
  for (int i = 0; i < TILES; ++i) {
#pragma unroll
    for (int j = 0; j < TILES; ++j) {
      const int gc = n0 + wn + j * 32 + col_l;
      if (gc >= N) continue;
      if (atomic) {
#pragma unroll
        for (int r = 0; r < 16; ++r) {
          const int gr = m0 + wm + i * 32 + (r & 3) + 8 * (r >> 2) + row_h;
          if (gr < M) atomicAdd(C + (int64_t)gr * ldc + gc, alpha * acc[i][j][r]);
        }
        continue;
      }
      const float bv = bias ? bias[gc] : 0.f;
#pragma unroll
      for (int r = 0; r < 16; ++r) {
        const int gr = m0 + wm + i * 32 + (r & 3) + 8 * (r >> 2) + row_h;
        if (gr < M) {
          float* o = C + (int64_t)gr * ldc + gc;
          float v = alpha * acc[i][j][r] + bv;
          if (beta != 0.f) v += beta * (*o);
          if (act == 1) v = fmaxf(v, 0.f);
          else if (act == 2) v = gate[(int64_t)gr * ldg + gc] > 0.f ? v : 0.f;
          *o = v;
        }
      }
    }
  }
}

template <bool TA, bool TB, int TILES, bool X3>
constexpr size_t gemm_smem_bytes() {
  if (X3) return 2 * 16 * (size_t)(GeoX<TILES>::template slots<!TA>() + GeoX<TILES>::template slots<TB>());
  return 2 * sizeof(float) * BK * (size_t)(Geo<TILES>::template ld<!TA>() + Geo<TILES>::template ld<TB>());
}

template <bool TA, bool TB, int TILES, bool X3, bool SEG = false>
__device__ __forceinline__ void gemm_block(void* smem, int M, int N, int K, int kbeg, float alpha, const float* __restrict__ A, int64_t lda,
                                           const float* __restrict__ B, int64_t ldb, float beta, float* __restrict__ C,
                                           int64_t ldc, const float* __restrict__ bias, bool vecA, bool vecB, int m0, int n0,
                                           bool atomic, float* colsum = nullptr, int act = 0, const float* __restrict__ gate = nullptr,
                                           int64_t ldg = 0, int nseg = 1, int64_t segA = 0, int64_t segB = 0) {
  const int tid = threadIdx.x, lane = tid & 63, w = tid >> 6;
  const int wm = (w >> 1) * 32 * TILES, wn = (w & 1) * 32 * TILES;

  f32x16 acc[TILES][TILES];
#ifdef PK2_GEMM_PROFILE
  const long long gp_t0 = wall_clock64();
#endif
  if constexpr (X3) {
    typedef u32x4_t (*StA)[GeoX<TILES>::template slots<!TA>()];
    typedef u32x4_t (*StB)[GeoX<TILES>::template slots<TB>()];
    StA Ax = reinterpret_cast<StA>(smem);
    StB Bx = reinterpret_cast<StB>(reinterpret_cast<u32x4_t*>(smem) + 2 * GeoX<TILES>::template slots<!TA>());
    if constexpr (!SEG) tile_mainloop_bf16x3<!TA, TB, TILES>(A, lda, B, ldb, m0, n0, kbeg, K, M, N, vecA, vecB, Ax, Bx, acc, n0 == 0 ? colsum : nullptr);
    else
      for (int sg = 0; sg < nseg; ++sg)
        tile_mainloop_bf16x3<!TA, TB, TILES>(A + sg * segA, lda, B + sg * segB, ldb, m0, n0, kbeg, K, M, N, vecA, vecB, Ax, Bx, acc, nullptr, sg == 0);
  } else {
    constexpr int LDA = Geo<TILES>::template ld<!TA>(), LDB = Geo<TILES>::template ld<TB>();
    typedef float (*StA)[BK * LDA];
    typedef float (*StB)[BK * LDB];
    StA As = reinterpret_cast<StA>(smem);
    StB Bs = reinterpret_cast<StB>(reinterpret_cast<float*>(smem) + 2 * BK * LDA);
    if constexpr (!SEG) tile_mainloop<!TA, TB, TILES>(A, lda, B, ldb, m0, n0, kbeg, K, M, N, vecA, vecB, As, Bs, acc);
    else
      for (int sg = 0; sg < nseg; ++sg)
        tile_mainloop<!TA, TB, TILES>(A + sg * segA, lda, B + sg * segB, ldb, m0, n0, kbeg, K, M, N, vecA, vecB, As, Bs, acc, sg == 0);
  }
#ifdef PK2_GEMM_PROFILE
  const long long gp_t1 = wall_clock64();
#endif
  gemm_store<TILES>(acc, M, N, alpha, beta, C, ldc, bias, m0, n0, wm, wn, atomic, act, gate, ldg);
#ifdef PK2_GEMM_PROFILE
  asm volatile("s_waitcnt vmcnt(0)" ::: "memory");
#ifndef PK2_GEMM_PROFILE_N
#define PK2_GEMM_PROFILE_N 4096
#define PK2_GEMM_PROFILE_K 1024
#define PK2_GEMM_PROFILE_EVERY 97
#endif
  if (tid == 0 && K == PK2_GEMM_PROFILE_K && N == PK2_GEMM_PROFILE_N && (blockIdx.x + blockIdx.y * gridDim.x) % PK2_GEMM_PROFILE_EVERY == 0) {
    unsigned xcc;
    asm volatile("s_getreg_b32 %0, hwreg(HW_REG_XCC_ID)" : "=s"(xcc));
    printf("gemm tile (%d,%d) of grid (%d,%d) tiles=%d xcc %u: start %lld main loop %lld epilogue %lld (10 ns ticks)\n", blockIdx.x, blockIdx.y,
           gridDim.x, gridDim.y, TILES, xcc & 7u, gp_t0, gp_t1 - gp_t0, wall_clock64() - gp_t1);
  }
#endif
}

template <bool TA, bool TB, int TILES, bool X3, bool SEG = false>
__global__ void __launch_bounds__(kGemmThreads, X3 ? PK2_GEMMX_WAVES : 3) gemm_f32_kernel(int M, int N, int K, float alpha,
                                                                const float* __restrict__ A, int64_t lda,
                                                                const float* __restrict__ B, int64_t ldb,
                                                                float beta, float* __restrict__ C, int64_t ldc,
                                                                const float* __restrict__ bias, bool vecA,
                                                                bool vecB, GemmBatch bt) {
  int kbeg = 0;
  {
    int z = blockIdx.z;
    if (bt.ksplit > 1) {
      kbeg = (z % bt.ksplit) * bt.klen;
      z /= bt.ksplit;
      K = min(K, kbeg + bt.klen);
    }
    const int i0 = z / bt.n1, i1 = z % bt.n1;
    A += i0 * bt.sA0 + i1 * bt.sA1;
    B += i0 * bt.sB0 + i1 * bt.sB1;
    C += i0 * bt.sC0 + i1 * bt.sC1;
  }
  __shared__ __attribute__((aligned(16))) char smem[gemm_smem_bytes<TA, TB, TILES, X3>()];
  gemm_block<TA, TB, TILES, X3, SEG>(smem, M, N, K, kbeg, alpha, A, lda, B, ldb, beta, C, ldc, bias, vecA, vecB,
                                blockIdx.y * Geo<TILES>::BMN, blockIdx.x * Geo<TILES>::BMN, bt.ksplit > 1, bt.colsum, bt.act, bt.gate,
                                bt.ldg, bt.nseg, bt.segA, bt.segB);
}

template <bool TA, bool TB, bool X3>
__global__ void __launch_bounds__(kGemmThreads, X3 ? PK2_GEMMX_WAVES : 3) gemm_f32_bands_kernel(int M, int N, int K, float alpha,
                                                                         const float* __restrict__ A, int64_t lda,
                                                                         const float* __restrict__ B, int64_t ldb,
                                                                         float beta, float* __restrict__ C, int64_t ldc,
                                                                         const float* __restrict__ bias, bool vecA,
                                                                         bool vecB, int nbig, int big_cols, int m_split,
                                                                         int small_cols) {
  const int b = blockIdx.x;
  __shared__ __attribute__((aligned(16))) char smem[std::max(gemm_smem_bytes<TA, TB, 2, X3>(), gemm_smem_bytes<TA, TB, 1, X3>())];
  if (b < nbig) {
    gemm_block<TA, TB, 2, X3>(smem, M, N, K, 0, alpha, A, lda, B, ldb, beta, C, ldc, bias, vecA, vecB, (b / big_cols) * 128,
                              (b % big_cols) * 128, false);
  } else {
    const int s = b - nbig;
    gemm_block<TA, TB, 1, X3>(smem, M, N, K, 0, alpha, A, lda, B, ldb, beta, C, ldc, bias, vecA, vecB, m_split + (s / small_cols) * 64,
                              (s % small_cols) * 64, false);
  }
}

__global__ void __launch_bounds__(256) gemm_prescale_kernel(int M, int N, float beta, float* __restrict__ C,
                                                            int64_t ldc, const float* __restrict__ bias, GemmBatch bt) {
  C += (blockIdx.z / bt.n1) * bt.sC0 + (blockIdx.z % bt.n1) * bt.sC1;
  const int n = blockIdx.x * 256 + threadIdx.x;
  if (n >= N) return;
  const float bv = bias ? bias[n] : 0.f;
  for (int m = blockIdx.y; m < M; m += gridDim.y) {
    float* o = C + (int64_t)m * ldc + n;
    *o = beta == 0.f ? bv : beta * (*o) + bv;
  }
}

__global__ void __launch_bounds__(256) colsum_kernel(const float* __restrict__ A, int64_t lda, int M, int N,
                                                     int rows_per_block, float* __restrict__ out) {
  __shared__ float red[4][64];
  const int n = blockIdx.x * 64 + (threadIdx.x & 63);
  const int part = threadIdx.x >> 6;
  const int m0 = blockIdx.y * rows_per_block, m1 = min(M, m0 + rows_per_block);
  float acc = 0.f;
  if (n < N)
    for (int m = m0 + part; m < m1; m += 4) acc += A[(int64_t)m * lda + n];
  red[part][threadIdx.x & 63] = acc;
  __syncthreads();
  if (part == 0 && n < N)
    atomicAdd(out + n, (red[0][threadIdx.x] + red[1][threadIdx.x]) + (red[2][threadIdx.x] + red[3][threadIdx.x]));
}

__global__ void scale_vec_kernel(float* v, int n, float beta) {
  const int i = blockIdx.x * blockDim.x + threadIdx.x;
  if (i < n) v[i] = beta == 0.f ? 0.f : beta * v[i];
}

}

using namespace pk2;

#ifndef PK2_GEMM_ARITH_DEFAULT
#define PK2_GEMM_ARITH_DEFAULT 1
#endif
extern "C" int pk2_colsum_f32(const float* A, int64_t lda, int32_t M, int32_t N, float beta, float* out, void* stream_);
static int g_gemm_arith = -1;
static int gemm_arith() {
  if (g_gemm_arith < 0) {
    const char* e = getenv("PK2_GEMM_ARITH");
    g_gemm_arith = e ? (strcmp(e, "f32") == 0 ? 0 : 1) : PK2_GEMM_ARITH_DEFAULT;
  }
  return g_gemm_arith;
}
extern "C" int pk2_gemm_set_arith(int32_t arith) {
  PK2_REQUIRE(arith == 0 || arith == 1, "gemm_set_arith: 0 = f32, 1 = bf16x3");
  g_gemm_arith = arith;
  return PK2_OK;
}
extern "C" int pk2_gemm_get_arith(void) { return gemm_arith(); }

#ifndef PK2_GEMM_MIN_KSLICE
#define PK2_GEMM_MIN_KSLICE 256
#endif
static int gemm_launch(int transa, int transb, int M, int N, int K, float alpha, const float* A, int64_t lda,
                       const float* B, int64_t ldb, float beta, float* C, int64_t ldc, const float* bias,
                       int n0, const GemmBatch& bt_in, bool aligned_strides, hipStream_t stream) {
  GemmBatch bt = bt_in;
  const bool x3 = gemm_arith() == 1;
  const bool vecA = aligned_strides && (reinterpret_cast<uintptr_t>(A) & 15) == 0 && (lda & 3) == 0;
  const bool vecB = aligned_strides && (reinterpret_cast<uintptr_t>(B) & 15) == 0 && (ldb & 3) == 0;
  const int64_t big_tiles = (int64_t)((N + 127) / 128) * ((M + 127) / 128) * n0 * bt.n1;
  const char* force = getenv("PK2_GEMM_TILES");
  int tiles = force ? atoi(force) : ((big_tiles >= 512 && K >= 256) ? 2 : 1);
  bt.ksplit = 1;
  bt.klen = K;
  const char* fsplit = getenv("PK2_GEMM_SPLITK");
  static const bool split_mid = [] { const char* e = getenv("PK2_GEMM_SPLIT_MID"); return !(e && atoi(e) == 0); }();
  const int deep_k = big_tiles <= 16 ? 1536 : 2048;
  static const bool split_fwd = [] { const char* e = getenv("PK2_GEMM_SPLIT_FWD"); return e && atoi(e) == 1; }();
  const bool forward_form = !transa && transb && !split_fwd;
  if (!forward_form && bt.act == 0 && bt.nseg == 1 && (big_tiles <= 256 || (split_mid && transa && !transb && big_tiles < 512)) && K >= deep_k && (!fsplit || atoi(fsplit) != 1)) {
    int ks = (int)std::min<int64_t>((768 + big_tiles - 1) / big_tiles, K / PK2_GEMM_MIN_KSLICE);
    if (big_tiles > 256) {
      double best = -1.0;
      for (int c = 2; c <= std::min(16, K / 1024); ++c) {
        const int64_t n = big_tiles * c;
        const double eff = (double)n / (double)((n + 511) / 512 * 512);
        if (eff >= best) { best = eff; ks = c; }
      }
    }
    if (fsplit && atoi(fsplit) > 1) ks = atoi(fsplit);
    if (ks > 1 && (int64_t)n0 * bt.n1 * ks <= 65535) {
      tiles = 2;
      bt.klen = ((K + ks - 1) / ks + BK - 1) / BK * BK;
      bt.ksplit = (K + bt.klen - 1) / bt.klen;
      if (beta != 1.f || bias)
        hipLaunchKernelGGL(gemm_prescale_kernel, dim3((N + 255) / 256, std::min(M, 256), n0 * bt.n1), dim3(256), 0,
                           stream, M, N, beta, C, ldc, bias, bt);
    }
  }
  auto launch = [&](int t, int m_off, int m_rows) {
    const int edge = 64 * t;
    const float* Ap = transa ? A + m_off : A + (int64_t)m_off * lda;
    float* Cp = C + (int64_t)m_off * ldc;
    dim3 grid((N + edge - 1) / edge, (m_rows + edge - 1) / edge, n0 * bt.n1 * bt.ksplit), block(kGemmThreads);
#define PK2_GEMM_T(TA, TB, T, X)                                                                                  \
  hipLaunchKernelGGL((gemm_f32_kernel<TA, TB, T, X>), grid, block, 0, stream, m_rows, N, K, alpha, Ap, lda, B, ldb, \
                     beta, Cp, ldc, bias, vecA, vecB, bt)
#define PK2_GEMM_SEG_T(TB, T, X)                                                                                  \
  hipLaunchKernelGGL((gemm_f32_kernel<false, TB, T, X, true>), grid, block, 0, stream, m_rows, N, K, alpha, Ap, lda, B, ldb, \
                     beta, Cp, ldc, bias, vecA, vecB, bt)
    if (bt.nseg > 1) {
      if (transb) { if (t == 2) { if (x3) PK2_GEMM_SEG_T(true, 2, true); else PK2_GEMM_SEG_T(true, 2, false); }
                    else        { if (x3) PK2_GEMM_SEG_T(true, 1, true); else PK2_GEMM_SEG_T(true, 1, false); } }
      else        { if (t == 2) { if (x3) PK2_GEMM_SEG_T(false, 2, true); else PK2_GEMM_SEG_T(false, 2, false); }
                    else        { if (x3) PK2_GEMM_SEG_T(false, 1, true); else PK2_GEMM_SEG_T(false, 1, false); } }
      return;
    }
#define PK2_GEMM(TA, TB)                                                                                          \
  do {                                                                                                            \
    if (t == 2) { if (x3) PK2_GEMM_T(TA, TB, 2, true); else PK2_GEMM_T(TA, TB, 2, false); }                       \
    else        { if (x3) PK2_GEMM_T(TA, TB, 1, true); else PK2_GEMM_T(TA, TB, 1, false); }                       \
  } while (0)
    if (!transa && !transb) PK2_GEMM(false, false);
    else if (!transa && transb) PK2_GEMM(false, true);
    else if (transa && !transb) PK2_GEMM(true, false);
    else PK2_GEMM(true, true);
#undef PK2_GEMM
#undef PK2_GEMM_T
#undef PK2_GEMM_SEG_T
  };
  int cus = 256;
  const char* band_env = getenv("PK2_GEMM_BANDS");
  const bool no_band = band_env && atoi(band_env) == 0;
  if (tiles == 2 && !no_band && bt.ksplit == 1 && n0 * bt.n1 == 1 && !force && !bt.colsum && bt.act == 0 && bt.nseg == 1 && (transa ? (lda & 3) == 0 : true)) {
    const int Cn = (N + 127) / 128, R = (M + 127) / 128, Cs = (N + 63) / 64;
    auto rounds = [&](int64_t n) { return (double)((n + cus - 1) / cus); };
    int best_r = R; double best = rounds((int64_t)R * Cn);
    for (int r = 0; r < R; ++r) {
      const int rest = M - r * 128;
      const double c = rounds((int64_t)r * Cn) + 0.3 * rounds((int64_t)((rest + 63) / 64) * Cs);
      if (c < best - 1e-9) { best = c; best_r = r; }
    }
    if (best_r < R) {
      static const bool one_launch = [] { const char* e = getenv("PK2_GEMM_BANDS_ONE"); return !(e && atoi(e) == 0); }();
      if (best_r > 0 && one_launch) {
        const int m_split = best_r * 128, small_rows = (M - m_split + 63) / 64;
        const int nbig = best_r * Cn;
        dim3 grid(nbig + small_rows * Cs), block(kGemmThreads);
#define PK2_GEMM_BANDS_X(TA, TB, X)                                                                                        \
  hipLaunchKernelGGL((gemm_f32_bands_kernel<TA, TB, X>), grid, block, 0, stream, M, N, K, alpha, A, lda, B, ldb, beta, C,   \
                     ldc, bias, vecA, vecB, nbig, Cn, m_split, Cs)
#define PK2_GEMM_BANDS(TA, TB) do { if (x3) PK2_GEMM_BANDS_X(TA, TB, true); else PK2_GEMM_BANDS_X(TA, TB, false); } while (0)
        if (!transa && !transb) PK2_GEMM_BANDS(false, false);
        else if (!transa && transb) PK2_GEMM_BANDS(false, true);
        else if (transa && !transb) PK2_GEMM_BANDS(true, false);
        else PK2_GEMM_BANDS(true, true);
#undef PK2_GEMM_BANDS
#undef PK2_GEMM_BANDS_X
        PK2_LAUNCH_CHECK();
        return PK2_OK;
      }
      if (best_r > 0) launch(2, 0, best_r * 128);
      launch(1, best_r * 128, M - best_r * 128);
      PK2_LAUNCH_CHECK();
      return PK2_OK;
    }
  }
  launch(tiles, 0, M);
  PK2_LAUNCH_CHECK();
  return PK2_OK;
}

extern "C" int pk2_gemm_f32(int32_t transa, int32_t transb, int32_t M, int32_t N, int32_t K, float alpha,
                            const float* A, int64_t lda, const float* B, int64_t ldb, float beta, float* C,
                            int64_t ldc, const float* bias, void* stream_) {
  PK2_REQUIRE(A && B && C && M > 0 && N > 0 && K > 0, "gemm_f32: bad args");
  GemmBatch bt{1, 0, 0, 0, 0, 0, 0, 1, 0};
  return gemm_launch(transa, transb, M, N, K, alpha, A, lda, B, ldb, beta, C, ldc, bias, 1, bt, true,
                     static_cast<hipStream_t>(stream_));
}

extern "C" int pk2_gemm_f32_act(int32_t transa, int32_t transb, int32_t M, int32_t N, int32_t K, float alpha,
                                const float* A, int64_t lda, const float* B, int64_t ldb, float beta, float* C,
                                int64_t ldc, const float* bias, int32_t act, const float* gate, int64_t ldg, void* stream_) {
  PK2_REQUIRE(A && B && C && M > 0 && N > 0 && K > 0, "gemm_f32_act: bad args");
  PK2_REQUIRE(act == 0 || act == 1 || (act == 2 && gate && ldg >= N), "gemm_f32_act: act is 0, 1 (ReLU) or 2 (gate, ldg >= N)");
  GemmBatch bt{1, 0, 0, 0, 0, 0, 0, 1, 0};
  bt.act = act; bt.gate = gate; bt.ldg = ldg;
  return gemm_launch(transa, transb, M, N, K, alpha, A, lda, B, ldb, beta, C, ldc, bias, 1, bt, true,
                     static_cast<hipStream_t>(stream_));
}

extern "C" int pk2_gemm_f32_seg(int32_t transa, int32_t transb, int32_t M, int32_t N, int32_t K, int32_t nseg, float alpha,
                                const float* A, int64_t lda, int64_t segA, const float* B, int64_t ldb, int64_t segB, float beta,
                                float* C, int64_t ldc, const float* bias, int32_t act, const float* gate, int64_t ldg,
                                void* stream_) {
  PK2_REQUIRE(A && B && C && M > 0 && N > 0 && K > 0 && nseg >= 1 && nseg <= 16, "gemm_f32_seg: bad args");
  PK2_REQUIRE(!transa, "gemm_f32_seg: A is row-major [M, K] (transa = 0)");
  PK2_REQUIRE(act == 0 || act == 1 || (act == 2 && gate && ldg >= N), "gemm_f32_seg: act is 0, 1 (ReLU) or 2 (gate, ldg >= N)");
  GemmBatch bt{1, 0, 0, 0, 0, 0, 0, 1, 0};
  bt.act = act; bt.gate = gate; bt.ldg = ldg;
  bt.nseg = nseg; bt.segA = segA; bt.segB = segB;
  const bool aligned = nseg == 1 || ((segA & 3) == 0 && (segB & 3) == 0);
  return gemm_launch(transa, transb, M, N, K, alpha, A, lda, B, ldb, beta, C, ldc, bias, 1, bt, aligned,
                     static_cast<hipStream_t>(stream_));
}

extern "C" int pk2_gemm_f32_tn_colsum(int32_t M, int32_t N, int32_t K, float alpha, const float* A, int64_t lda, const float* B,
                                      int64_t ldb, float beta, float* C, int64_t ldc, float* colsum, void* stream_) {
  PK2_REQUIRE(A && B && C && colsum && M > 0 && N > 0 && K > 0, "gemm_f32_tn_colsum: bad args");
  GemmBatch bt{1, 0, 0, 0, 0, 0, 0, 1, 0};
  static const bool fuse_env = [] { const char* e = getenv("PK2_GEMM_FUSE_COLSUM"); return !(e && atoi(e) == 0); }();
  const bool fuse = fuse_env && gemm_arith() == 1;
  if (fuse) bt.colsum = colsum;
  int rc = gemm_launch(1, 0, M, N, K, alpha, A, lda, B, ldb, beta, C, ldc, nullptr, 1, bt, true, static_cast<hipStream_t>(stream_));
  if (rc || fuse) return rc;
  return pk2_colsum_f32(A, lda, K, M, 1.0f, colsum, stream_);
}

extern "C" int pk2_gemm_f32_batched(int32_t transa, int32_t transb, int32_t M, int32_t N, int32_t K, float alpha,
                                    const float* A, int64_t lda, int64_t strideA0, int64_t strideA1,
                                    const float* B, int64_t ldb, int64_t strideB0, int64_t strideB1, float beta,
                                    float* C, int64_t ldc, int64_t strideC0, int64_t strideC1, int32_t n0,
                                    int32_t n1, void* stream_) {
  PK2_REQUIRE(A && B && C && M > 0 && N > 0 && K > 0 && n0 > 0 && n1 > 0 && (int64_t)n0 * n1 <= 65535,
              "gemm_f32_batched: bad args");
  GemmBatch bt{n1, strideA0, strideA1, strideB0, strideB1, strideC0, strideC1, 1, 0};
  const bool aligned = ((strideA0 | strideA1 | strideB0 | strideB1) & 3) == 0;
  return gemm_launch(transa, transb, M, N, K, alpha, A, lda, B, ldb, beta, C, ldc, nullptr, n0, bt, aligned,
                     static_cast<hipStream_t>(stream_));
}

extern "C" int pk2_colsum_f32(const float* A, int64_t lda, int32_t M, int32_t N, float beta, float* out,
                              void* stream_) {
  PK2_REQUIRE(A && out && M > 0 && N > 0, "colsum_f32: bad args");
  hipStream_t stream = static_cast<hipStream_t>(stream_);
  if (beta != 1.f) hipLaunchKernelGGL(scale_vec_kernel, dim3((N + 255) / 256), dim3(256), 0, stream, out, N, beta);
  const int col_blocks = (N + 63) / 64;
  const int splits = std::max(1, std::min((M + 63) / 64, 1024 / col_blocks));
  const int rows_per_block = (M + splits - 1) / splits;
  hipLaunchKernelGGL(colsum_kernel, dim3(col_blocks, (M + rows_per_block - 1) / rows_per_block), dim3(256), 0, stream,
                     A, lda, M, N, rows_per_block, out);
  PK2_LAUNCH_CHECK();
  return PK2_OK;
}
```

pykaldi2_amd/csrc/gemm_tile.h:

```cpp
#pragma once
#include <type_traits>

#include "common.h"

namespace pk2 {

typedef float f32x16 __attribute__((ext_vector_type(16)));

__device__ __forceinline__ void lds_barrier() { asm volatile("s_waitcnt lgkmcnt(0)\n\ts_barrier" ::: "memory"); }

constexpr int BK = 16;
constexpr int kGemmThreads = 256;
template <int TILES> struct Geo {
  static constexpr int BMN = 64 * TILES;
  static constexpr int LD = BMN + 4;
  static constexpr int LDK = BMN + 2;
  static constexpr int LPK = 16 * TILES;
  template <bool KCONTIG> static constexpr int ld() { return KCONTIG ? LDK : LD; }
};

template <bool KCONTIG, int TILES>
__device__ __forceinline__ void load_slab(const float* __restrict__ base, int64_t ld, int r0, int k0,
                                          int R, int K, bool vec, float4 (&reg)[TILES]) {
  const int tid = threadIdx.x;
#pragma unroll
  for (int h = 0; h < TILES; ++h) {
    int r, k;
    if (KCONTIG) { r = (tid >> 2) + h * 64; k = (tid & 3) * 4; }
    else         { k = tid / Geo<TILES>::LPK + h * (kGemmThreads / Geo<TILES>::LPK); r = (tid % Geo<TILES>::LPK) * 4; }
    const int gr = r0 + r, gk = k0 + k;
    float4 v = make_float4(0.f, 0.f, 0.f, 0.f);
    if (KCONTIG) {
      if (gr < R) {
        const float* p = base + (int64_t)gr * ld + gk;
        if (vec && gk + 3 < K) {
          v = *reinterpret_cast<const float4*>(p);
        } else {
          if (gk + 0 < K) v.x = p[0];
          if (gk + 1 < K) v.y = p[1];
          if (gk + 2 < K) v.z = p[2];
          if (gk + 3 < K) v.w = p[3];
        }
      }
    } else {
      if (gk < K) {
        const float* p = base + (int64_t)gk * ld + gr;
        if (vec && gr + 3 < R) {
          v = *reinterpret_cast<const float4*>(p);
        } else {
          if (gr + 0 < R) v.x = p[0];
          if (gr + 1 < R) v.y = p[1];
          if (gr + 2 < R) v.z = p[2];
          if (gr + 3 < R) v.w = p[3];
        }
      }
    }
    reg[h] = v;
  }
}


template <bool KCONTIG, int TILES>
__device__ __forceinline__ void slab_pointers(const float* __restrict__ base, int64_t ld, int r0, int k0, int R,
                                              const float* (&ptr)[TILES], int64_t* step) {
  const int tid = threadIdx.x;
#pragma unroll
  for (int h = 0; h < TILES; ++h) {
    if (KCONTIG) {
      const int r = (tid >> 2) + h * 64, k = (tid & 3) * 4;
      ptr[h] = base + (int64_t)min(r0 + r, R - 1) * ld + k0 + k;
    } else {
      const int k = tid / Geo<TILES>::LPK + h * (kGemmThreads / Geo<TILES>::LPK), r = (tid % Geo<TILES>::LPK) * 4;
      ptr[h] = base + (int64_t)(k0 + k) * ld + min(r0 + r, R - 4);
    }
  }
  *step = KCONTIG ? (int64_t)BK : (int64_t)BK * ld;
}
template <int TILES>
__device__ __forceinline__ void load_slab_fast(const float* const (&ptr)[TILES], int64_t off, float4 (&reg)[TILES]) {
#pragma unroll
  for (int h = 0; h < TILES; ++h) reg[h] = *reinterpret_cast<const float4*>(ptr[h] + off);
}

template <bool KCONTIG, int TILES>
__device__ __forceinline__ void store_slab(float* __restrict__ tile, const float4 (&reg)[TILES]) {
  const int tid = threadIdx.x;
  constexpr int LD = Geo<TILES>::template ld<KCONTIG>();
#pragma unroll
  for (int h = 0; h < TILES; ++h) {
    if (KCONTIG) {
      const int r = (tid >> 2) + h * 64, k = (tid & 3) * 4;
      tile[(k + 0) * LD + r] = reg[h].x;
      tile[(k + 1) * LD + r] = reg[h].y;
      tile[(k + 2) * LD + r] = reg[h].z;
      tile[(k + 3) * LD + r] = reg[h].w;
    } else {
      const int k = tid / Geo<TILES>::LPK + h * (kGemmThreads / Geo<TILES>::LPK), r = (tid % Geo<TILES>::LPK) * 4;
      *reinterpret_cast<float4*>(&tile[k * LD + r]) = reg[h];
    }
  }
}

template <int I, int N, class F>
__device__ __forceinline__ void static_for(F&& f) {
  if constexpr (I < N) {
    f(std::integral_constant<int, I>());
    static_for<I + 1, N>(f);
  }
}

template <bool KCA, bool KCB, int TILES>
__device__ __forceinline__ void tile_mainloop(const float* __restrict__ A, int64_t lda, const float* __restrict__ B, int64_t ldb,
                                              int m0, int n0, int kbeg, int K, int M, int N, bool vecA, bool vecB,
                                              float (*As)[BK * Geo<TILES>::template ld<KCA>()],
                                              float (*Bs)[BK * Geo<TILES>::template ld<KCB>()],
                                              f32x16 (&acc)[TILES][TILES], bool zero_acc = true) {
  constexpr int BM = Geo<TILES>::BMN, BN = Geo<TILES>::BMN;
  constexpr int LDA = Geo<TILES>::template ld<KCA>(), LDB = Geo<TILES>::template ld<KCB>();
  const int lane = threadIdx.x & 63, w = threadIdx.x >> 6;
  const int wm = (w >> 1) * 32 * TILES, wn = (w & 1) * 32 * TILES;
  if (zero_acc) {
#pragma unroll
    for (int i = 0; i < TILES; ++i)
#pragma unroll
      for (int j = 0; j < TILES; ++j)
#pragma unroll
        for (int r = 0; r < 16; ++r) acc[i][j][r] = 0.f;
  }
  const int kq = lane >> 5, li = lane & 31;
#ifndef PK2_GEMM_DEPTH2
#define PK2_GEMM_DEPTH2 2
#endif
#ifndef PK2_GEMM_DEPTH1
#define PK2_GEMM_DEPTH1 6
#endif
  constexpr int DEPTH = TILES == 1 ? PK2_GEMM_DEPTH1 : PK2_GEMM_DEPTH2;
  static_assert(DEPTH % 2 == 0, "an even number of register stages (the LDS buffer is the stage's parity)");
  float4 ra[DEPTH][TILES], rb[DEPTH][TILES];
  const int nk = (K - kbeg + BK - 1) / BK;
  const bool interior = vecA && vecB && (m0 + BM <= M || KCA || ((M & 3) == 0 && M >= 4)) &&
                        (n0 + BN <= N || KCB || ((N & 3) == 0 && N >= 4));
  const float* pa[TILES]; const float* pb[TILES];
  int64_t stepA = 0, stepB = 0;
  slab_pointers<KCA, TILES>(A, lda, m0, kbeg, M, pa, &stepA);
  slab_pointers<KCB, TILES>(B, ldb, n0, kbeg, N, pb, &stepB);
#ifndef PK2_GEMM_HOIST
#define PK2_GEMM_HOIST 8
#endif
  auto multiply = [&](auto C_) {
    constexpr int cur = decltype(C_)::value;
    constexpr int GRP = TILES == 1 ? PK2_GEMM_HOIST : 1;
#pragma unroll
    for (int k0 = 0; k0 < BK / 2; k0 += GRP) {
      float a[GRP][TILES], b[GRP][TILES];
#pragma unroll
      for (int g = 0; g < GRP; ++g) {
#pragma unroll
        for (int i = 0; i < TILES; ++i) a[g][i] = As[cur][(2 * (k0 + g) + kq) * LDA + wm + i * 32 + li];
#pragma unroll
        for (int j = 0; j < TILES; ++j) b[g][j] = Bs[cur][(2 * (k0 + g) + kq) * LDB + wn + j * 32 + li];
      }
      if (GRP > 1) __builtin_amdgcn_sched_barrier(0);
#pragma unroll
      for (int g = 0; g < GRP; ++g)
#pragma unroll
        for (int i = 0; i < TILES; ++i)
#pragma unroll
          for (int j = 0; j < TILES; ++j)
            acc[i][j] = __builtin_amdgcn_mfma_f32_32x32x2f32(a[g][i], b[g][j], acc[i][j], 0, 0, 0);
    }
  };
  auto pipeline = [&](int n, auto fetch) {
    if (n <= 0) return;
#pragma unroll
    for (int i = 0; i < DEPTH; ++i) fetch(min(i, n - 1), ra[i], rb[i]);
    store_slab<KCA, TILES>(As[0], ra[0]);
    store_slab<KCB, TILES>(Bs[0], rb[0]);
    lds_barrier();
    fetch(min(DEPTH, n - 1), ra[0], rb[0]);
    auto slab_step = [&](int kt, auto P) {
      constexpr int st = decltype(P)::value, cur = st & 1, nxt = 1 - cur, sn = (st + 1) % DEPTH;
      multiply(std::integral_constant<int, cur>());
      if (kt + 1 < n) {
        store_slab<KCA, TILES>(As[nxt], ra[sn]);
        store_slab<KCB, TILES>(Bs[nxt], rb[sn]);
      }
      lds_barrier();
      if (kt + 1 + DEPTH < n) fetch(kt + 1 + DEPTH, ra[sn], rb[sn]);
    };
    auto steady_step = [&](int kt, auto P) {
      constexpr int st = decltype(P)::value, cur = st & 1, nxt = 1 - cur, sn = (st + 1) % DEPTH;
      multiply(std::integral_constant<int, cur>());
      store_slab<KCA, TILES>(As[nxt], ra[sn]);
      store_slab<KCB, TILES>(Bs[nxt], rb[sn]);
      lds_barrier();
      fetch(min(kt + 1 + DEPTH, n - 1), ra[sn], rb[sn]);
    };
    int kt = 0;
    for (; kt + DEPTH <= n; kt += DEPTH)
      static_for<0, DEPTH>([&](auto S) { steady_step(kt + decltype(S)::value, S); });
    if (kt < n)
      static_for<0, DEPTH>([&](auto S) { if (kt + decltype(S)::value < n) slab_step(kt + decltype(S)::value, S); });
  };
  if (interior) {
    const int nk_fast = (K - kbeg) / BK;
    pipeline(nk_fast, [&](int ks, float4 (&xa)[TILES], float4 (&xb)[TILES]) {
      load_slab_fast<TILES>(pa, ks * stepA, xa);
      load_slab_fast<TILES>(pb, ks * stepB, xb);
    });
    if (nk > nk_fast) {
      load_slab<KCA, TILES>(A, lda, m0, kbeg + nk_fast * BK, M, K, vecA, ra[0]);
      load_slab<KCB, TILES>(B, ldb, n0, kbeg + nk_fast * BK, N, K, vecB, rb[0]);
      store_slab<KCA, TILES>(As[0], ra[0]);
      store_slab<KCB, TILES>(Bs[0], rb[0]);
      lds_barrier();
      multiply(std::integral_constant<int, 0>());
      lds_barrier();
    }
  } else {
    pipeline(nk, [&](int ks, float4 (&xa)[TILES], float4 (&xb)[TILES]) {
      load_slab<KCA, TILES>(A, lda, m0, kbeg + ks * BK, M, K, vecA, xa);
      load_slab<KCB, TILES>(B, ldb, n0, kbeg + ks * BK, N, K, vecB, xb);
    });
  }
}

}
```

pykaldi2_amd/fbank.py:

```python
import ctypes as C
import os

import numpy as np
import torch

from . import _lib

def mel_filterbank(sr=16000, n_fft=512, n_mels=80, fmin=0.0, fmax=7690.0):
    def hz2mel(f):
        return 2595.0 * np.log10(1.0 + f / 700.0)

    def mel2hz(m):
        return 700.0 * (10.0 ** (m / 2595.0) - 1.0)
    fftfreqs = np.linspace(0, sr / 2, n_fft // 2 + 1)
    mel_f = mel2hz(np.linspace(hz2mel(fmin), hz2mel(fmax), n_mels + 2))
    fdiff = np.diff(mel_f)
    ramps = np.subtract.outer(mel_f, fftfreqs)
    w = np.zeros((n_mels, n_fft // 2 + 1))
    for i in range(n_mels):
        w[i] = np.maximum(0, np.minimum(-ramps[i] / fdiff[i], ramps[i + 2] / fdiff[i + 1]))
    w *= (2.0 / (mel_f[2:n_mels + 2] - mel_f[:n_mels]))[:, None]
    return w.astype(np.float32)


def load_mel(path):
    with open(path) as f:
        rows = [np.asarray([np.float32(v) for v in line.rstrip("\n").split(",")]) for line in f if line.strip()]
    mel = np.vstack(rows).astype(np.float32)
    assert mel.shape == (80, 257), mel.shape
    return mel


def num_frames(num_samples):
    return int(_lib.lib().pk2_fbank_num_frames(int(num_samples)))


class FbankExtractor:
    def __init__(self, mel=None):
        mel = mel_filterbank() if mel is None else np.ascontiguousarray(mel, dtype=np.float32)
        h = C.c_void_p()
        _lib.check(_lib.lib().pk2_fbank_create(_lib.ptr(mel), C.byref(h)))
        self._h = h

    def __del__(self):
        try:
            if getattr(self, "_h", None):
                _lib.lib().pk2_fbank_destroy(self._h)
                self._h = None
        except Exception:
            pass

    def __call__(self, wav, wav_lengths, apply_cmn=True):
        _lib.require_gpu()
        assert wav.is_cuda and wav.dtype == torch.float32 and wav.is_contiguous()
        n = len(wav_lengths)
        wav_off = np.zeros(n + 1, dtype=np.int64)
        wav_off[1:] = np.cumsum(wav_lengths)
        frames = [num_frames(l) for l in wav_lengths]
        row_off_h = np.zeros(n + 1, dtype=np.int64)
        row_off_h[1:] = np.cumsum(frames)
        row_off = torch.from_numpy(row_off_h).pin_memory().to(wav.device, non_blocking=True)
        feats = torch.empty(int(row_off_h[-1]), 80, dtype=torch.float32, device=wav.device)
        _lib.check(_lib.lib().pk2_fbank_compute(self._h, _lib.ptr(wav), _lib.ptr(wav_off), n, _lib.ptr(feats),
                                                _lib.ptr(row_off), 1 if apply_cmn else 0,
                                                _lib.stream_ptr(wav.device)))
        return feats, frames, row_off

    @staticmethod
    def pad_roll_subsample(feats, row_off, frames, shift=0, subsample=1, time_major=False):
        n = len(frames)
        max_t = int(max(frames))
        out_t = (max_t - 1) // subsample + 1
        shape = (out_t, n, 80) if time_major else (n, out_t, 80)
        x = torch.empty(*shape, dtype=torch.float32, device=feats.device)
        _lib.check(_lib.lib().pk2_pad_roll_subsample(_lib.ptr(feats), _lib.ptr(row_off), n, max_t, int(shift),
                                                     int(subsample), _lib.ptr(x), out_t, 1 if time_major else 0,
                                                     _lib.stream_ptr(feats.device)))
        return x


def utt2seg(feats, seg_len, seg_shift):
    T = feats.shape[0]
    n_seg = (T - seg_len) // seg_shift + 1 if T >= seg_len else 0
    if n_seg <= 0:
        return feats.new_zeros((0, seg_len) + tuple(feats.shape[1:]))
    inner = int(np.prod(feats.shape[1:])) if feats.dim() > 1 else 1
    f = feats.contiguous()
    view = f.as_strided((n_seg, seg_len) + tuple(f.shape[1:]), (seg_shift * inner, inner) + tuple(f.stride()[1:]))
    return view.contiguous()


class _MvnState:

    def __init__(self, mean_vec, std_vec):
        self.mean_vec, self.std_vec, self.mean_norm, self.var_norm = mean_vec, std_vec, True, True


class GlobalMeanVarianceNormalization:

    def __init__(self, mean_vec, std_vec):
        self.mean_vec = np.ascontiguousarray(mean_vec, dtype=np.float32).reshape(1, -1)
        self.std_vec = np.ascontiguousarray(std_vec, dtype=np.float32).reshape(1, -1)
        self._dev = None

    @classmethod
    def from_stats(cls, mean_stats, var_stats, n_frame):
        mean = np.asarray(mean_stats, dtype=np.float32).reshape(-1, 1) / n_frame
        std = np.sqrt(np.asarray(var_stats, dtype=np.float32).reshape(-1, 1) / n_frame - mean ** 2)
        std = np.maximum(std, 1e-2)
        std[np.isnan(std)] = 1.0
        std[np.isinf(std)] = 1.0
        return cls(mean.T, std.T)

    @classmethod
    def load(cls, path):
        import pickle

        class _Bag:
            def __setstate__(self, state):
                self.__dict__.update(state)

        class _Unpickler(pickle.Unpickler):
            def find_class(self, module, name):
                if module.startswith("numpy") or module in ("builtins", "collections", "_codecs"):
                    return super().find_class(module, name)
                return _Bag

        with open(path, "rb") as f:
            o = _Unpickler(f).load()
        mean = np.asarray(o.mean_vec, np.float32).reshape(1, -1)
        std = np.asarray(o.std_vec, np.float32).reshape(1, -1)
        if not getattr(o, "mean_norm", True):
            mean = np.zeros_like(mean)
        if not getattr(o, "var_norm", True):
            std = np.ones_like(std)
        return cls(mean, std)

    def save(self, path):
        import pickle
        with open(path, "wb") as f:
            pickle.dump(_MvnState(self.mean_vec, self.std_vec), f, pickle.HIGHEST_PROTOCOL)

    @classmethod
    def estimate(cls, source, extractor, device, n_sample_to_use=2000, apply_cmn=True, batch=8):
        s1 = torch.zeros(80, dtype=torch.float64, device=device)
        s2 = torch.zeros(80, dtype=torch.float64, device=device)
        n_frame, seen = 0, 0
        while seen < n_sample_to_use:
            utts = [source.draw() for _ in range(min(batch, n_sample_to_use - seen))]
            seen += len(utts)
            lens = [u[0].shape[0] for u in utts]
            wav = torch.from_numpy(np.concatenate([u[0] for u in utts])).to(device)
            feats, frames, _ = extractor(wav, lens, apply_cmn=apply_cmn)
            f64 = feats.double()
            s1 += f64.sum(0)
            s2 += (f64 * f64).sum(0)
            n_frame += int(sum(frames))
        return cls.from_stats(s1.cpu().numpy(), s2.cpu().numpy(), n_frame)

    def __call__(self, x):
        return self.apply_on_tensor(x)

    def apply_on_tensor(self, x):
        _lib.require_gpu()
        assert x.is_cuda and x.dtype == torch.float32 and x.is_contiguous() and x.shape[-1] == self.mean_vec.shape[1]
        if self._dev is None or self._dev[0].device != x.device:
            self._dev = (torch.from_numpy(self.mean_vec).to(x.device), torch.from_numpy(self.std_vec).to(x.device))
        y = torch.empty_like(x)
        _lib.check(_lib.lib().pk2_mvn_apply(_lib.ptr(x), _lib.ptr(self._dev[0]), _lib.ptr(self._dev[1]),
                                            x.numel() // x.shape[-1], x.shape[-1], _lib.ptr(y),
                                            _lib.stream_ptr(x.device)))
        return y
```

pykaldi2_amd/lstm.py:

```python
import math
import ctypes
import os

import torch
import torch.nn as nn

from . import _lib


def _gemm(ta, tb, M, N, K, A, lda, B, ldb, C, ldc, bias=None, alpha=1.0, beta=0.0):
    _lib.check(_lib.lib().pk2_gemm_f32(int(ta), int(tb), M, N, K, alpha, A, lda, B, ldb, beta, C, ldc,
                                       bias, _lib.stream_ptr()))


def _p(t, off_floats=0):
    import ctypes
    return ctypes.c_void_p(t.data_ptr() + 4 * off_floats)


class _LSTMParams(nn.Module):

    def __init__(self, input_size, hidden_size, num_layers, bidirectional):
        super().__init__()
        self.input_size, self.hidden_size = input_size, hidden_size
        self.num_layers, self.bidirectional = num_layers, bidirectional
        D = 2 if bidirectional else 1
        H = hidden_size
        for layer in range(num_layers):
            for d in range(D):
                in_size = input_size if layer == 0 else H * D
                sfx = "_reverse" if d == 1 else ""
                self.register_parameter("weight_ih_l%d%s" % (layer, sfx), nn.Parameter(torch.empty(4 * H, in_size)))
                self.register_parameter("weight_hh_l%d%s" % (layer, sfx), nn.Parameter(torch.empty(4 * H, H)))
                self.register_parameter("bias_ih_l%d%s" % (layer, sfx), nn.Parameter(torch.empty(4 * H)))
                self.register_parameter("bias_hh_l%d%s" % (layer, sfx), nn.Parameter(torch.empty(4 * H)))
        stdv = 1.0 / math.sqrt(H) if H > 0 else 0
        for w in self.parameters():
            nn.init.uniform_(w, -stdv, stdv)


class _LinearParams(nn.Module):

    def __init__(self, in_features, out_features):
        super().__init__()
        self.weight = nn.Parameter(torch.empty(out_features, in_features))
        self.bias = nn.Parameter(torch.empty(out_features))
        nn.init.kaiming_uniform_(self.weight, a=math.sqrt(5))
        bound = 1 / math.sqrt(in_features) if in_features > 0 else 0
        nn.init.uniform_(self.bias, -bound, bound)


class _LstmAmFunction(torch.autograd.Function):

    @staticmethod
    def forward(ctx, x_tm, model, *params):
        m = model
        T, B, Din = x_tm.shape
        H, D, Lr = m.hidden_size, m.num_dirs, m.num_layers
        dev = x_tm.device
        L = _lib.lib()
        sp = _lib.stream_ptr()
        rows = T * B
        saved = []
        seeds = []
        inp = x_tm.contiguous()
        for l in range(Lr):
            w_ih, w_hh, b_ih, b_hh = m._layer_views(l)
            in_size = inp.shape[-1]
            y = torch.empty(T, B, D * H, device=dev, dtype=torch.float32)
            gates = torch.empty(D, T, B, 4 * H, device=dev, dtype=torch.float32)
            cells = torch.empty(D, T, B, H, device=dev, dtype=torch.float32)
            nws = L.pk2_lstm_fwd_workspace_floats(B, H, D)
            ws = torch.empty(nws, device=dev, dtype=torch.float32) if nws else None
            gx_done = ctypes.c_int32(0)
            _lib.check(L.pk2_lstm_layer_fwd_xproj(None, _p(w_hh), _p(b_hh), B, T, H, D, _p(y), _p(gates), _p(cells),
                                                  _p(ws) if ws is not None else None, _p(inp), in_size, _p(w_ih), _p(b_ih),
                                                  ctypes.byref(gx_done), sp))
            if not gx_done.value:
                gx = torch.empty(T, B, D * 4 * H, device=dev, dtype=torch.float32)
                _gemm(0, 1, rows, D * 4 * H, in_size, _p(inp), in_size, _p(w_ih), in_size, _p(gx), D * 4 * H,
                      bias=_p(b_ih))
                _lib.check(L.pk2_lstm_layer_fwd(_p(gx), _p(w_hh), _p(b_hh), B, T, H, D, _p(y), _p(gates), _p(cells),
                                                _p(ws) if ws is not None else None, sp))
            saved.append((inp, y, gates, cells))
            inp = y
            if m.dropout > 0 and m.training and l + 1 < Lr:
                seed = int(torch.empty((), dtype=torch.int64).random_().item()) & 0x7FFFFFFFFFFFFFFF
                seeds.append(seed)
                inp = torch.empty_like(y)
                _lib.check(L.pk2_dropout_f32(_p(y), _p(inp), y.numel(), float(m.dropout), seed, sp))
            else:
                seeds.append(None)
        P = m.output_size
        logits = torch.empty(T, B, P, device=dev, dtype=torch.float32)
        _gemm(0, 1, rows, P, D * H, _p(inp), D * H, _p(m.output_layer.weight), D * H, _p(logits), P,
              bias=_p(m.output_layer.bias))
        ctx.model = m
        ctx.saved = saved
        ctx.seeds = seeds
        ctx.shape = (T, B, Din)
        ctx.need_dx = x_tm.requires_grad
        return logits

    @staticmethod
    def backward(ctx, dlogits):
        m = ctx.model
        T, B, Din = ctx.shape
        H, D, Lr, P = m.hidden_size, m.num_dirs, m.num_layers, m.output_size
        L = _lib.lib()
        sp = _lib.stream_ptr()
        rows = T * B
        dev = dlogits.device
        dlogits = dlogits.contiguous()
        gflat = m._grad_flat()
        gflat.zero_()
        views = m._grad_views(gflat)
        y_last = ctx.saved[-1][1]
        main = torch.cuda.current_stream(dev)
        side = m._side_stream(dev) if os.environ.get("PK2_SIDE_STREAM") == "1" else main

        def on_side(fn, *tensors):
            ev = torch.cuda.Event()
            ev.record(main)
            with torch.cuda.stream(side):
                side.wait_event(ev)
                fn()
            for t_ in tensors:
                t_.record_stream(side)

        gw, gb = views["output_layer.weight"], views["output_layer.bias"]
        dy = torch.empty(T, B, D * H, device=dev, dtype=torch.float32)
        _gemm(0, 0, rows, D * H, P, _p(dlogits), P, _p(m.output_layer.weight), D * H, _p(dy), D * H)

        def out_grads():
            _lib.check(L.pk2_gemm_f32_tn_colsum(P, D * H, rows, 1.0, _p(dlogits), P, _p(y_last), D * H, 1.0, _p(gw), D * H, _p(gb),
                                                _lib.stream_ptr()))
            m._bucket_ready("output_layer")
        on_side(out_grads, dlogits, y_last)
        scratch = torch.empty(L.pk2_lstm_bwd_scratch_floats(B, H, D), device=dev, dtype=torch.float32)
        dx = None
        for l in range(Lr - 1, -1, -1):
            inp, y, gates, cells = ctx.saved[l]
            in_size = inp.shape[-1]
            w_ih, w_hh, b_ih, b_hh = m._layer_views(l)
            gw_ih, gw_hh, gb_ih, gb_hh = m._layer_views(l, gflat)
            dgx = torch.empty(T, B, D * 4 * H, device=dev, dtype=torch.float32)
            bias_done = ctypes.c_int32(0)
            whh_done = ctypes.c_int32(0)
            nws = L.pk2_lstm_bwd_wgrad_workspace_floats(B, H, D)
            wgrad_ws = torch.empty(nws, device=dev, dtype=torch.float32) if nws else None
            _lib.check(L.pk2_lstm_layer_bwd_wgrad(_p(dy), _p(w_hh), _p(gates), _p(cells), _p(y), B, T, H, D, _p(dgx), _p(scratch),
                                                  _p(gb_ih), _p(gb_hh), _p(gw_hh), _p(wgrad_ws) if nws else None,
                                                  ctypes.byref(bias_done), ctypes.byref(whh_done), sp))
            G = D * 4 * H

            def layer_grads(dgx=dgx, inp=inp, y=y, in_size=in_size, gw_ih=gw_ih, gw_hh=gw_hh, gb_ih=gb_ih,
                            gb_hh=gb_hh, l=l, bias_done=bool(bias_done.value), whh_done=bool(whh_done.value)):
                if not bias_done:
                    _lib.check(L.pk2_gemm_f32_tn_colsum(G, in_size, rows, 1.0, _p(dgx), G, _p(inp), in_size, 1.0, _p(gw_ih), in_size,
                                                        _p(gb_ih), _lib.stream_ptr()))
                    gb_hh.copy_(gb_ih)
                else:
                    _gemm(1, 0, G, in_size, rows, _p(dgx), G, _p(inp), in_size, _p(gw_ih), in_size, beta=1.0)
                if T > 1 and not whh_done:
                    k = (T - 1) * B
                    if D == 2:
                        _lib.check(L.pk2_gemm_f32_batched(1, 0, 4 * H, H, k, 1.0, _p(dgx, B * G), G, 4 * H - B * G, 0,
                                                          _p(y), D * H, B * D * H + H, 0, 1.0, _p(gw_hh), H,
                                                          4 * H * H, 0, 2, 1, _lib.stream_ptr()))
                    else:
                        _gemm(1, 0, 4 * H, H, k, _p(dgx, B * G), G, _p(y), D * H, _p(gw_hh), H, beta=1.0)
                m._bucket_ready("lstm.l%d" % l)
            if l > 0 or ctx.need_dx:
                dprev = torch.empty(T, B, in_size, device=dev, dtype=torch.float32)
                ev = torch.cuda.Event()
                ev.record(main)
                _gemm(0, 0, rows, in_size, G, _p(dgx), G, _p(w_ih), in_size, _p(dprev), in_size)
                with torch.cuda.stream(side):
                    side.wait_event(ev)
                    layer_grads()
                for t_ in (dgx, inp, y):
                    t_.record_stream(side)
                if l > 0:
                    dy = dprev
                    if ctx.seeds[l - 1] is not None:
                        _lib.check(L.pk2_dropout_f32(_p(dy), _p(dy), dy.numel(), float(m.dropout), ctx.seeds[l - 1], sp))
                else:
                    dx = dprev
            else:
                on_side(layer_grads, dgx, inp, y)
        main.wait_stream(side)
        params = dict(m.named_parameters())
        for name in m._param_names:
            p, v = params[name], views[name]
            if p.grad is None or p.grad.data_ptr() != v.data_ptr():
                p.grad = v
        ctx.saved = None
        return (dx, None) + (None,) * len(m._param_names)


class LSTMAM(nn.Module):
    def __init__(self, input_size, output_size, hidden_size, num_layers, dropout, bidirectional):
        super().__init__()
        self.input_size = input_size
        self.output_size = output_size
        self.hidden_size = hidden_size
        self.num_layers = num_layers
        self.dropout = dropout
        self.bidirectional = bidirectional
        self.num_dirs = 2 if bidirectional else 1
        self.output_layer = _LinearParams(hidden_size * self.num_dirs, output_size)
        self.lstm = _LSTMParams(input_size, hidden_size, num_layers, bidirectional)
        self._param_names = [n for n, _ in self.named_parameters()]
        self._flat = None
        self._gflat = None
        self._layout = None
        self._bucket_hook = None

    def _flat_order(self):
        order = ["output_layer.weight", "output_layer.bias"]
        sfx = ["", "_reverse"][:self.num_dirs]
        for l in range(self.num_layers):
            for kind in ("weight_ih", "weight_hh", "bias_ih", "bias_hh"):
                for s in sfx:
                    order.append("lstm.%s_l%d%s" % (kind, l, s))
        return order

    def _ensure_flat(self):
        params = dict(self.named_parameters())
        first = params["output_layer.weight"]
        if self._flat is not None and self._flat.device == first.device and all(
                params[n].data_ptr() == self._flat.data_ptr() + 4 * off for n, (off, _) in self._layout.items()):
            return
        order = self._flat_order()
        layout, off = {}, 0
        for n in order:
            cnt = params[n].numel()
            layout[n] = (off, cnt)
            off += (cnt + 63) // 64 * 64
        flat = torch.zeros(off, dtype=torch.float32, device=first.device)
        for n in order:
            o, cnt = layout[n]
            flat[o:o + cnt].copy_(params[n].data.reshape(-1))
            params[n].data = flat[o:o + cnt].view(params[n].shape)
        self._flat, self._layout = flat, layout
        self._gflat = None
        self._buckets = {}
        names = order
        def span(prefixes):
            sel = [layout[n] for n in names if any(n.startswith(p) for p in prefixes)]
            lo = min(o for o, _ in sel)
            hi = max((o + c + 63) // 64 * 64 for o, c in sel)
            return lo, hi
        self._buckets["output_layer"] = span(["output_layer."])
        for l in range(self.num_layers):
            self._buckets["lstm.l%d" % l] = span(["lstm.%s_l%d" % (k, l) for k in ("weight_ih", "weight_hh", "bias_ih", "bias_hh")])

    def flat_parameters(self):
        self._ensure_flat()
        return self._flat, self._grad_flat()

    def _grad_flat(self):
        self._ensure_flat()
        if self._gflat is None or self._gflat.device != self._flat.device:
            self._gflat = torch.zeros_like(self._flat)
        return self._gflat

    def _grad_views(self, gflat):
        params = dict(self.named_parameters())
        return {n: gflat[o:o + c].view(params[n].shape) for n, (o, c) in self._layout.items()}

    def _layer_views(self, l, flat=None):
        flat = self._flat if flat is None else flat
        D, H = self.num_dirs, self.hidden_size
        in_size = self.input_size if l == 0 else H * D
        def seg(kind, cols):
            o, _ = self._layout["lstm.%s_l%d" % (kind, l)]
            n = D * 4 * H * cols
            return flat[o:o + n].view(D * 4 * H, cols) if cols > 1 else flat[o:o + D * 4 * H]
        return seg("weight_ih", in_size), seg("weight_hh", H), seg("bias_ih", 1), seg("bias_hh", 1)

    def _side_stream(self, dev):
        st = getattr(self, "_side", None)
        if st is None or st.device != dev:
            k = int(os.environ.get("PK2_SIDE_CU_PER_XCD", "0"))
            if k > 0:
                h = ctypes.c_void_p()
                with torch.cuda.device(dev):
                    _lib.check(_lib.lib().pk2_stream_create_cu_mask(k, ctypes.byref(h)))
                st = torch.cuda.ExternalStream(h.value, device=dev)
                self._side_handle = h
            else:
                st = torch.cuda.Stream(device=dev)
            self._side = st
        return st

    def _bucket_ready(self, name):
        if self._bucket_hook is not None:
            lo, hi = self._buckets[name]
            self._bucket_hook(name, self._gflat[lo:hi])

    def forward_time_major(self, x_tm):
        _lib.require_gpu()
        assert x_tm.is_cuda and x_tm.dtype == torch.float32
        self._ensure_flat()
        D, H = self.num_dirs, self.hidden_size
        for l in range(self.num_layers):
            in_size = self.input_size if l == 0 else H * D
            assert (4 * H * in_size) % 64 == 0 and (4 * H * H) % 64 == 0 and (4 * H) % 64 == 0
        params = [p for _, p in self.named_parameters()]
        return _LstmAmFunction.apply(x_tm, self, *params)

    def forward(self, data):
        x_tm = data.transpose(0, 1).contiguous()
        return self.forward_time_major(x_tm).transpose(0, 1).contiguous()
```

Before: 4834.

## Skip padded frames in output-layer GEMMs using a valid-row map

Sequence lengths are attached to padded features and used to build a permutation of valid (time, batch) rows. The output-layer forward GEMM, the input-gradient GEMM and the weight-gradient GEMM then compute only valid rows through row-mapped load and store paths, and the padded rows are zeroed. This removes matrix work on padding frames at the cost of indirect gathers, a host-built map copied to the device, and extra kernel variants. It only takes effect when lengths reach the model, via fbank's pad_roll_subsample or an explicit argument.

```diff
diff --git a/include/pk2hip.h b/include/pk2hip.h
--- a/include/pk2hip.h
+++ b/include/pk2hip.h
@@ -351,6 +351,14 @@
 int pk2_gemm_get_arith(void);
 int pk2_gemm_f32_tn_colsum(int32_t M, int32_t N, int32_t K, float alpha, const float* A, int64_t lda, const float* B,
                            int64_t ldb, float beta, float* C, int64_t ldc, float* colsum, void* stream);
+int pk2_gemm_f32_rows(int32_t transb, int32_t M_total, int32_t N, int32_t K, float alpha, const float* A, int64_t lda,
+                      const float* B, int64_t ldb, float beta, float* C, int64_t ldc, const float* bias,
+                      const int32_t* rmap, int32_t Mv, void* stream);
+int pk2_gemm_f32_tn_colsum_rows(int32_t M, int32_t N, int32_t K_total, float alpha, const float* A, int64_t lda, const float* B,
+                                int64_t ldb, float beta, float* C, int64_t ldc, float* colsum, const int32_t* rmap, int32_t Kv,
+                                void* stream);
+int pk2_rows_zero(float* X, int64_t ldx, int32_t N, const int32_t* rows, int32_t n, void* stream);
+int pk2_rows_pack(const float* X, int64_t ldx, int32_t N, const int32_t* rows, int32_t n, float* out, int64_t ldo, void* stream);
 int pk2_colsum_f32(const float* A, int64_t lda, int32_t M, int32_t N, float beta, float* out,
                    void* stream);
 
diff --git a/pykaldi2_amd/_lib.py b/pykaldi2_amd/_lib.py
--- a/pykaldi2_amd/_lib.py
+++ b/pykaldi2_amd/_lib.py
@@ -234,6 +234,10 @@
     "pk2_gemm_f32_batched": (C.c_int, [_i32, _i32, _i32, _i32, _i32, _f32, _vp, _i64, _i64, _i64, _vp, _i64, _i64, _i64,
                                        _f32, _vp, _i64, _i64, _i64, _i32, _i32, _vp]),
     "pk2_gemm_f32_tn_colsum": (C.c_int, [_i32, _i32, _i32, _f32, _vp, _i64, _vp, _i64, _f32, _vp, _i64, _vp, _vp]),
+    "pk2_gemm_f32_rows": (C.c_int, [_i32, _i32, _i32, _i32, _f32, _vp, _i64, _vp, _i64, _f32, _vp, _i64, _vp, _vp, _i32, _vp]),
+    "pk2_gemm_f32_tn_colsum_rows": (C.c_int, [_i32, _i32, _i32, _f32, _vp, _i64, _vp, _i64, _f32, _vp, _i64, _vp, _vp, _i32, _vp]),
+    "pk2_rows_zero": (C.c_int, [_vp, _i64, _i32, _vp, _i32, _vp]),
+    "pk2_rows_pack": (C.c_int, [_vp, _i64, _i32, _vp, _i32, _vp, _i64, _vp]),
     "pk2_gemm_set_arith": (C.c_int, [_i32]),
     "pk2_gemm_get_arith": (C.c_int, []),
     "pk2_layernorm_fwd": (C.c_int, [_vp, _vp, _vp, _vp, _i64, _i32, _f32, _vp, _vp, _vp, _vp, _vp]),
diff --git a/pykaldi2_amd/csrc/gemm_bf16x3.h b/pykaldi2_amd/csrc/gemm_bf16x3.h
--- a/pykaldi2_amd/csrc/gemm_bf16x3.h
+++ b/pykaldi2_amd/csrc/gemm_bf16x3.h
@@ -55,24 +55,52 @@
   }
 };
 
-template <bool KC, int TILES>
+template <bool KC, int TILES, int MAP = kMapNone>
 __device__ __forceinline__ void xslab_pointers(const PieceMap<KC, TILES>& pm, const float* __restrict__ base, int64_t ld, int r0,
-                                               int k0, int R, const float* (&ptr)[2], int64_t* step) {
+                                               int k0, int R, const float* (&ptr)[2], int64_t* step, const int* __restrict__ rmap = nullptr) {
+  static_assert(MAP == kMapNone || (MAP == kMapRows && KC) || (MAP == kMapK && !KC), "which operand layout a map applies to");
 #pragma unroll
   for (int h = 0; h < 2; ++h) {
+    if constexpr (MAP == kMapRows) ptr[h] = base + (int64_t)rmap[min(r0 + pm.row[h], R - 1)] * ld + k0 + pm.k[h];
+    else if constexpr (MAP == kMapK) ptr[h] = base + min(r0 + pm.row[h], R - 4);
+    else
     if (KC) ptr[h] = base + (int64_t)min(r0 + pm.row[h], R - 1) * ld + k0 + pm.k[h];
     else    ptr[h] = base + (int64_t)(k0 + pm.k[h]) * ld + min(r0 + pm.row[h], R - 4);
   }
   *step = KC ? (int64_t)GeoX<TILES>::BK : (int64_t)GeoX<TILES>::BK * ld;
 }
 
-template <bool KC, int TILES>
+template <bool KC, int TILES, int MAP = kMapNone>
 __device__ __forceinline__ void xload_general(const PieceMap<KC, TILES>& pm, const float* __restrict__ base, int64_t ld, int r0,
-                                              int k0, int R, int K, bool vec, float4 (&reg)[2]) {
+                                              int k0, int R, int K, bool vec, float4 (&reg)[2], const int* __restrict__ rmap = nullptr) {
+  static_assert(MAP == kMapNone || (MAP == kMapRows && KC) || (MAP == kMapK && !KC), "which operand layout a map applies to");
 #pragma unroll
   for (int h = 0; h < 2; ++h) {
     const int gr = r0 + pm.row[h], gk = k0 + pm.k[h];
     float4 v = make_float4(0.f, 0.f, 0.f, 0.f);
+    if constexpr (MAP == kMapRows) {
+      if (gr < R) {
+        const float* p = base + (int64_t)rmap[gr] * ld + gk;
+        if (vec && gk + 3 < K) v = *reinterpret_cast<const float4*>(p);
+        else {
+          if (gk + 0 < K) v.x = p[0];
+          if (gk + 1 < K) v.y = p[1];
+          if (gk + 2 < K) v.z = p[2];
+          if (gk + 3 < K) v.w = p[3];
+        }
+      }
+    } else if constexpr (MAP == kMapK) {
+      if (gk < K) {
+        const float* p = base + (int64_t)rmap[gk] * ld + gr;
+        if (vec && gr + 3 < R) v = *reinterpret_cast<const float4*>(p);
+        else {
+          if (gr + 0 < R) v.x = p[0];
+          if (gr + 1 < R) v.y = p[1];
+          if (gr + 2 < R) v.z = p[2];
+          if (gr + 3 < R) v.w = p[3];
+        }
+      }
+    } else
     if (KC) {
       if (gr < R) {
         const float* p = base + (int64_t)gr * ld + gk;
@@ -133,13 +161,15 @@
   }
 }
 
-template <bool KCA, bool KCB, int TILES>
+template <bool KCA, bool KCB, int TILES, int MAP = kMapNone>
 __device__ __forceinline__ void tile_mainloop_bf16x3(const float* __restrict__ A, int64_t lda, const float* __restrict__ B, int64_t ldb,
                                                      int m0, int n0, int kbeg, int K, int M, int N, bool vecA, bool vecB,
                                                      u32x4_t (*As)[GeoX<TILES>::template slots<KCA>()],
                                                      u32x4_t (*Bs)[GeoX<TILES>::template slots<KCB>()],
                                                      f32x16 (&acc)[TILES][TILES], float* __restrict__ colsum = nullptr,
-                                                     bool zero_acc = true) {
+                                                     bool zero_acc = true, const int* __restrict__ rmap = nullptr) {
+  static_assert(MAP == kMapNone || (MAP == kMapRows && KCA) || (MAP == kMapK && !KCA && !KCB), "kMapRows: rows of a k-contiguous A; kMapK: both operands row-contiguous");
+  constexpr int MAPB = MAP == kMapK ? kMapK : kMapNone;
   typedef GeoX<TILES> G;
   constexpr int BM = G::BMN, BN = G::BMN, XBK = G::BK, NKG = G::NKG;
   constexpr int SPA = G::template sp<KCA>(), SPB = G::template sp<KCB>();
@@ -173,8 +203,8 @@
                         (n0 + BN <= N || KCB || ((N & 3) == 0 && N >= 4));
   const float* pa[2]; const float* pb[2];
   int64_t stepA = 0, stepB = 0;
-  xslab_pointers<KCA, TILES>(pma, A, lda, m0, kbeg, M, pa, &stepA);
-  xslab_pointers<KCB, TILES>(pmb, B, ldb, n0, kbeg, N, pb, &stepB);
+  xslab_pointers<KCA, TILES, MAP>(pma, A, lda, m0, kbeg, M, pa, &stepA, rmap);
+  xslab_pointers<KCB, TILES, MAPB>(pmb, B, ldb, n0, kbeg, N, pb, &stepB, rmap);
   int sa[TILES], sb[TILES];
 #pragma unroll
   for (int i = 0; i < TILES; ++i) sa[i] = kq * SPA + G::template slot<KCA>(wm + i * 32 + li);
@@ -243,6 +273,23 @@
   };
   if (interior) {
     const int nk_fast = (K - kbeg) / XBK;
+    if constexpr (MAP == kMapK) {
+      int mk[2];
+#pragma unroll
+      for (int h = 0; h < 2; ++h) mk[h] = nk_fast > 0 ? rmap[kbeg + pma.k[h]] : 0;
+      pipeline(nk_fast, [&](int ks, float4 (&xa)[2], float4 (&xb)[2]) {
+        int nm[2];
+        const int kn = kbeg + min(ks + 1, nk_fast - 1) * XBK;
+#pragma unroll
+        for (int h = 0; h < 2; ++h) nm[h] = rmap[kn + pma.k[h]];
+#pragma unroll
+        for (int h = 0; h < 2; ++h) xa[h] = *reinterpret_cast<const float4*>(pa[h] + (int64_t)mk[h] * lda);
+#pragma unroll
+        for (int h = 0; h < 2; ++h) xb[h] = *reinterpret_cast<const float4*>(pb[h] + (int64_t)mk[h] * ldb);
+#pragma unroll
+        for (int h = 0; h < 2; ++h) mk[h] = nm[h];
+      });
+    } else
     pipeline(nk_fast, [&](int ks, float4 (&xa)[2], float4 (&xb)[2]) {
 #ifdef PK2_X3_DBG_NOLOAD
       ks = 0;
@@ -253,8 +300,8 @@
       for (int h = 0; h < 2; ++h) xb[h] = *reinterpret_cast<const float4*>(pb[h] + ks * stepB);
     });
     if (nk > nk_fast) {
-      xload_general<KCA, TILES>(pma, A, lda, m0, kbeg + nk_fast * XBK, M, K, vecA, ra[0]);
-      xload_general<KCB, TILES>(pmb, B, ldb, n0, kbeg + nk_fast * XBK, N, K, vecB, rb[0]);
+      xload_general<KCA, TILES, MAP>(pma, A, lda, m0, kbeg + nk_fast * XBK, M, K, vecA, ra[0], rmap);
+      xload_general<KCB, TILES, MAPB>(pmb, B, ldb, n0, kbeg + nk_fast * XBK, N, K, vecB, rb[0], rmap);
       store_a(As[0], ra[0]);
       xstore<KCB, TILES>(pmb, Bs[0], rb[0]);
       lds_barrier();
@@ -263,8 +310,8 @@
     }
   } else {
     pipeline(nk, [&](int ks, float4 (&xa)[2], float4 (&xb)[2]) {
-      xload_general<KCA, TILES>(pma, A, lda, m0, kbeg + ks * XBK, M, K, vecA, xa);
-      xload_general<KCB, TILES>(pmb, B, ldb, n0, kbeg + ks * XBK, N, K, vecB, xb);
+      xload_general<KCA, TILES, MAP>(pma, A, lda, m0, kbeg + ks * XBK, M, K, vecA, xa, rmap);
+      xload_general<KCB, TILES, MAPB>(pmb, B, ldb, n0, kbeg + ks * XBK, N, K, vecB, xb, rmap);
     });
   }
   if constexpr (!KCA) {
diff --git a/pykaldi2_amd/csrc/gemm_f32.hip b/pykaldi2_amd/csrc/gemm_f32.hip
--- a/pykaldi2_amd/csrc/gemm_f32.hip
+++ b/pykaldi2_amd/csrc/gemm_f32.hip
@@ -15,10 +15,11 @@
 #ifndef PK2_GEMMX_WAVES
 #define PK2_GEMMX_WAVES 2
 #endif
-template <int TILES>
+template <int TILES, bool RMAP = false>
 __device__ __forceinline__ void gemm_store(const f32x16 (&acc)[TILES][TILES], int M, int N, float alpha, float beta, float* __restrict__ C,
                                            int64_t ldc, const float* __restrict__ bias, int m0, int n0, int wm, int wn, bool atomic,
-                                           int act = 0, const float* __restrict__ gate = nullptr, int64_t ldg = 0) {
+                                           int act = 0, const float* __restrict__ gate = nullptr, int64_t ldg = 0,
+                                           const int* __restrict__ rmap = nullptr) {
   const int lane = threadIdx.x & 63;
   const int col_l = lane & 31, row_h = 4 * (lane >> 5);
 #pragma unroll
@@ -31,6 +32,8 @@
 #pragma unroll
         for (int r = 0; r < 16; ++r) {
           const int gr = m0 + wm + i * 32 + (r & 3) + 8 * (r >> 2) + row_h;
+          if constexpr (RMAP) { if (gr < M) atomicAdd(C + (int64_t)rmap[gr] * ldc + gc, alpha * acc[i][j][r]); }
+          else
           if (gr < M) atomicAdd(C + (int64_t)gr * ldc + gc, alpha * acc[i][j][r]);
         }
         continue;
@@ -39,6 +42,14 @@
 #pragma unroll
       for (int r = 0; r < 16; ++r) {
         const int gr = m0 + wm + i * 32 + (r & 3) + 8 * (r >> 2) + row_h;
+        if constexpr (RMAP) {
+          if (gr < M) {
+            float* o = C + (int64_t)rmap[gr] * ldc + gc;
+            float v = alpha * acc[i][j][r] + bv;
+            if (beta != 0.f) v += beta * (*o);
+            *o = v;
+          }
+        } else
         if (gr < M) {
           float* o = C + (int64_t)gr * ldc + gc;
           float v = alpha * acc[i][j][r] + bv;
@@ -58,12 +69,14 @@
   return 2 * sizeof(float) * BK * (size_t)(Geo<TILES>::template ld<!TA>() + Geo<TILES>::template ld<TB>());
 }
 
-template <bool TA, bool TB, int TILES, bool X3, bool SEG = false>
+template <bool TA, bool TB, int TILES, bool X3, bool SEG = false, int MAP = kMapNone>
 __device__ __forceinline__ void gemm_block(void* smem, int M, int N, int K, int kbeg, float alpha, const float* __restrict__ A, int64_t lda,
                                            const float* __restrict__ B, int64_t ldb, float beta, float* __restrict__ C,
                                            int64_t ldc, const float* __restrict__ bias, bool vecA, bool vecB, int m0, int n0,
                                            bool atomic, float* colsum = nullptr, int act = 0, const float* __restrict__ gate = nullptr,
-                                           int64_t ldg = 0, int nseg = 1, int64_t segA = 0, int64_t segB = 0) {
+                                           int64_t ldg = 0, int nseg = 1, int64_t segA = 0, int64_t segB = 0,
+                                           const int* __restrict__ rmap = nullptr) {
+  static_assert(MAP == kMapNone || !SEG, "a mapped product has one segment");
   const int tid = threadIdx.x, lane = tid & 63, w = tid >> 6;
   const int wm = (w >> 1) * 32 * TILES, wn = (w & 1) * 32 * TILES;
 
@@ -76,6 +89,8 @@
     typedef u32x4_t (*StB)[GeoX<TILES>::template slots<TB>()];
     StA Ax = reinterpret_cast<StA>(smem);
     StB Bx = reinterpret_cast<StB>(reinterpret_cast<u32x4_t*>(smem) + 2 * GeoX<TILES>::template slots<!TA>());
+    if constexpr (MAP != kMapNone) tile_mainloop_bf16x3<!TA, TB, TILES, MAP>(A, lda, B, ldb, m0, n0, kbeg, K, M, N, vecA, vecB, Ax, Bx, acc, n0 == 0 ? colsum : nullptr, true, rmap);
+    else
     if constexpr (!SEG) tile_mainloop_bf16x3<!TA, TB, TILES>(A, lda, B, ldb, m0, n0, kbeg, K, M, N, vecA, vecB, Ax, Bx, acc, n0 == 0 ? colsum : nullptr);
     else
       for (int sg = 0; sg < nseg; ++sg)
@@ -86,6 +101,8 @@
     typedef float (*StB)[BK * LDB];
     StA As = reinterpret_cast<StA>(smem);
     StB Bs = reinterpret_cast<StB>(reinterpret_cast<float*>(smem) + 2 * BK * LDA);
+    if constexpr (MAP != kMapNone) tile_mainloop<!TA, TB, TILES, MAP>(A, lda, B, ldb, m0, n0, kbeg, K, M, N, vecA, vecB, As, Bs, acc, true, rmap);
+    else
     if constexpr (!SEG) tile_mainloop<!TA, TB, TILES>(A, lda, B, ldb, m0, n0, kbeg, K, M, N, vecA, vecB, As, Bs, acc);
     else
       for (int sg = 0; sg < nseg; ++sg)
@@ -94,6 +111,8 @@
 #ifdef PK2_GEMM_PROFILE
   const long long gp_t1 = wall_clock64();
 #endif
+  if constexpr (MAP == kMapRows) gemm_store<TILES, true>(acc, M, N, alpha, beta, C, ldc, bias, m0, n0, wm, wn, atomic, 0, nullptr, 0, rmap);
+  else
   gemm_store<TILES>(acc, M, N, alpha, beta, C, ldc, bias, m0, n0, wm, wn, atomic, act, gate, ldg);
 #ifdef PK2_GEMM_PROFILE
   asm volatile("s_waitcnt vmcnt(0)" ::: "memory");
@@ -157,6 +176,91 @@
   }
 }
 
+template <bool TA, bool TB, int TILES, bool X3, int MAP>
+__global__ void __launch_bounds__(kGemmThreads, X3 ? PK2_GEMMX_WAVES : 3) gemm_f32_rows_kernel(int M, int N, int K, float alpha,
+                                                                const float* __restrict__ A, int64_t lda,
+                                                                const float* __restrict__ B, int64_t ldb,
+                                                                float beta, float* __restrict__ C, int64_t ldc,
+                                                                const float* __restrict__ bias, bool vecA, bool vecB,
+                                                                int ksplit, int klen, float* __restrict__ colsum,
+                                                                const int* __restrict__ rmap) {
+  int kbeg = 0;
+  if (ksplit > 1) {
+    kbeg = blockIdx.z * klen;
+    K = min(K, kbeg + klen);
+  }
+  __shared__ __attribute__((aligned(16))) char smem[gemm_smem_bytes<TA, TB, TILES, X3>()];
+  gemm_block<TA, TB, TILES, X3, false, MAP>(smem, M, N, K, kbeg, alpha, A, lda, B, ldb, beta, C, ldc, bias, vecA, vecB,
+                                            blockIdx.y * Geo<TILES>::BMN, blockIdx.x * Geo<TILES>::BMN, ksplit > 1, colsum, 0, nullptr, 0,
+                                            1, 0, 0, rmap);
+}
+
+template <bool TB, bool X3>
+__global__ void __launch_bounds__(kGemmThreads, X3 ? PK2_GEMMX_WAVES : 3) gemm_f32_rows_bands_kernel(int M, int N, int K, float alpha,
+                                                                         const float* __restrict__ A, int64_t lda,
+                                                                         const float* __restrict__ B, int64_t ldb,
+                                                                         float beta, float* __restrict__ C, int64_t ldc,
+                                                                         const float* __restrict__ bias, bool vecA,
+                                                                         bool vecB, int nbig, int big_cols, int m_split,
+                                                                         int small_cols, const int* __restrict__ rmap) {
+  const int b = blockIdx.x;
+  __shared__ __attribute__((aligned(16))) char smem[std::max(gemm_smem_bytes<false, TB, 2, X3>(), gemm_smem_bytes<false, TB, 1, X3>())];
+  if (b < nbig) {
+    gemm_block<false, TB, 2, X3, false, kMapRows>(smem, M, N, K, 0, alpha, A, lda, B, ldb, beta, C, ldc, bias, vecA, vecB, (b / big_cols) * 128,
+                                                  (b % big_cols) * 128, false, nullptr, 0, nullptr, 0, 1, 0, 0, rmap);
+  } else {
+    const int s = b - nbig;
+    gemm_block<false, TB, 1, X3, false, kMapRows>(smem, M, N, K, 0, alpha, A, lda, B, ldb, beta, C, ldc, bias, vecA, vecB,
+                                                  m_split + (s / small_cols) * 64, (s % small_cols) * 64, false, nullptr, 0, nullptr, 0, 1,
+                                                  0, 0, rmap);
+  }
+}
+
+__global__ void __launch_bounds__(256) gemm_prescale_rows_kernel(int M, int N, float beta, float* __restrict__ C, int64_t ldc,
+                                                                 const float* __restrict__ bias, const int* __restrict__ rmap) {
+  const int n = blockIdx.x * 256 + threadIdx.x;
+  if (n >= N) return;
+  const float bv = bias ? bias[n] : 0.f;
+  for (int m = blockIdx.y; m < M; m += gridDim.y) {
+    float* o = C + (int64_t)rmap[m] * ldc + n;
+    *o = beta == 0.f ? bv : beta * (*o) + bv;
+  }
+}
+
+__global__ void __launch_bounds__(256) colsum_rows_kernel(const float* __restrict__ A, int64_t lda, int M, int N, int rows_per_block,
+                                                          float* __restrict__ out, const int* __restrict__ rmap) {
+  __shared__ float red[4][64];
+  const int n = blockIdx.x * 64 + (threadIdx.x & 63);
+  const int part = threadIdx.x >> 6;
+  const int m0 = blockIdx.y * rows_per_block, m1 = min(M, m0 + rows_per_block);
+  float acc = 0.f;
+  if (n < N)
+    for (int m = m0 + part; m < m1; m += 4) acc += A[(int64_t)rmap[m] * lda + n];
+  red[part][threadIdx.x & 63] = acc;
+  __syncthreads();
+  if (part == 0 && n < N)
+    atomicAdd(out + n, (red[0][threadIdx.x] + red[1][threadIdx.x]) + (red[2][threadIdx.x] + red[3][threadIdx.x]));
+}
+
+template <bool PACK>
+__global__ void __launch_bounds__(256) rows_zero_or_pack_kernel(float* __restrict__ X, int64_t ldx, int N, const int* __restrict__ rows,
+                                                                int n, float* __restrict__ out, int64_t ldo, bool vec) {
+  for (int i = blockIdx.y; i < n; i += gridDim.y) {
+    float* x = X + (int64_t)rows[i] * ldx;
+    if (vec) {
+      for (int c = (blockIdx.x * 256 + threadIdx.x) * 4; c < N; c += gridDim.x * 1024) {
+        if (PACK) *reinterpret_cast<float4*>(out + (int64_t)i * ldo + c) = *reinterpret_cast<const float4*>(x + c);
+        else *reinterpret_cast<float4*>(x + c) = make_float4(0.f, 0.f, 0.f, 0.f);
+      }
+    } else {
+      for (int c = blockIdx.x * 256 + threadIdx.x; c < N; c += gridDim.x * 256) {
+        if (PACK) out[(int64_t)i * ldo + c] = x[c];
+        else x[c] = 0.f;
+      }
+    }
+  }
+}
+
 __global__ void __launch_bounds__(256) gemm_prescale_kernel(int M, int N, float beta, float* __restrict__ C,
                                                             int64_t ldc, const float* __restrict__ bias, GemmBatch bt) {
   C += (blockIdx.z / bt.n1) * bt.sC0 + (blockIdx.z % bt.n1) * bt.sC1;
@@ -217,7 +321,8 @@
 #endif
 static int gemm_launch(int transa, int transb, int M, int N, int K, float alpha, const float* A, int64_t lda,
                        const float* B, int64_t ldb, float beta, float* C, int64_t ldc, const float* bias,
-                       int n0, const GemmBatch& bt_in, bool aligned_strides, hipStream_t stream) {
+                       int n0, const GemmBatch& bt_in, bool aligned_strides, hipStream_t stream,
+                       const int* rmap = nullptr, int map = kMapNone) {
   GemmBatch bt = bt_in;
   const bool x3 = gemm_arith() == 1;
   const bool vecA = aligned_strides && (reinterpret_cast<uintptr_t>(A) & 15) == 0 && (lda & 3) == 0;
@@ -232,8 +337,20 @@
   const int deep_k = big_tiles <= 16 ? 1536 : 2048;
   static const bool split_fwd = [] { const char* e = getenv("PK2_GEMM_SPLIT_FWD"); return e && atoi(e) == 1; }();
   const bool forward_form = !transa && transb && !split_fwd;
-  if (!forward_form && bt.act == 0 && bt.nseg == 1 && (big_tiles <= 256 || (split_mid && transa && !transb && big_tiles < 512)) && K >= deep_k && (!fsplit || atoi(fsplit) != 1)) {
+  static const bool rows_slices = [] { const char* e = getenv("PK2_GEMM_ROWS_SLICES"); return !(e && atoi(e) == 0); }();
+  const bool rows_rule = map != kMapNone && rows_slices && !forward_form && !fsplit && !force && big_tiles >= 64 && big_tiles < 512 && K >= 1024;
+  if (rows_rule || (!forward_form && bt.act == 0 && bt.nseg == 1 && (big_tiles <= 256 || (split_mid && transa && !transb && big_tiles < 512)) && K >= deep_k && (!fsplit || atoi(fsplit) != 1))) {
     int ks = (int)std::min<int64_t>((768 + big_tiles - 1) / big_tiles, K / PK2_GEMM_MIN_KSLICE);
+    if (rows_rule) {
+      double best = -1.0;
+      ks = 1;
+      for (int c = 1; c <= std::min(16, K / PK2_GEMM_MIN_KSLICE); ++c) {
+        const int64_t n = big_tiles * c;
+        const double eff = (double)n / (double)((n + 511) / 512 * 512);
+        if (eff >= 0.9) { ks = c; break; }
+        if (eff > best) { best = eff; ks = c; }
+      }
+    } else
     if (big_tiles > 256) {
       double best = -1.0;
       for (int c = 2; c <= std::min(16, K / 1024); ++c) {
@@ -247,7 +364,10 @@
       tiles = 2;
       bt.klen = ((K + ks - 1) / ks + BK - 1) / BK * BK;
       bt.ksplit = (K + bt.klen - 1) / bt.klen;
-      if (beta != 1.f || bias)
+      if ((beta != 1.f || bias) && map == kMapRows)
+        hipLaunchKernelGGL(gemm_prescale_rows_kernel, dim3((N + 255) / 256, std::min(M, 256)), dim3(256), 0, stream, M, N, beta, C, ldc,
+                           bias, rmap);
+      else if (beta != 1.f || bias)
         hipLaunchKernelGGL(gemm_prescale_kernel, dim3((N + 255) / 256, std::min(M, 256), n0 * bt.n1), dim3(256), 0,
                            stream, M, N, beta, C, ldc, bias, bt);
     }
@@ -263,6 +383,22 @@
 #define PK2_GEMM_SEG_T(TB, T, X)                                                                                  \
   hipLaunchKernelGGL((gemm_f32_kernel<false, TB, T, X, true>), grid, block, 0, stream, m_rows, N, K, alpha, Ap, lda, B, ldb, \
                      beta, Cp, ldc, bias, vecA, vecB, bt)
+    if (map != kMapNone) {
+#define PK2_GEMM_ROWS_T(TA, TB, T, X, MP)                                                                                  \
+  hipLaunchKernelGGL((gemm_f32_rows_kernel<TA, TB, T, X, MP>), grid, block, 0, stream, m_rows, N, K, alpha, A, lda, B, ldb, \
+                     beta, C, ldc, bias, vecA, vecB, bt.ksplit, bt.klen, bt.colsum, rmap)
+#define PK2_GEMM_ROWS(TA, TB, MP)                                                                                      \
+  do {                                                                                                                 \
+    if (t == 2) { if (x3) PK2_GEMM_ROWS_T(TA, TB, 2, true, MP); else PK2_GEMM_ROWS_T(TA, TB, 2, false, MP); }          \
+    else        { if (x3) PK2_GEMM_ROWS_T(TA, TB, 1, true, MP); else PK2_GEMM_ROWS_T(TA, TB, 1, false, MP); }          \
+  } while (0)
+      if (map == kMapK) PK2_GEMM_ROWS(true, false, kMapK);
+      else if (transb) PK2_GEMM_ROWS(false, true, kMapRows);
+      else PK2_GEMM_ROWS(false, false, kMapRows);
+#undef PK2_GEMM_ROWS
+#undef PK2_GEMM_ROWS_T
+      return;
+    }
     if (bt.nseg > 1) {
       if (transb) { if (t == 2) { if (x3) PK2_GEMM_SEG_T(true, 2, true); else PK2_GEMM_SEG_T(true, 2, false); }
                     else        { if (x3) PK2_GEMM_SEG_T(true, 1, true); else PK2_GEMM_SEG_T(true, 1, false); } }
@@ -297,6 +433,24 @@
     }
     if (best_r < R) {
       static const bool one_launch = [] { const char* e = getenv("PK2_GEMM_BANDS_ONE"); return !(e && atoi(e) == 0); }();
+      if (best_r > 0 && map == kMapRows) {
+        const int m_split = best_r * 128, small_rows = (M - m_split + 63) / 64;
+        const int nbig = best_r * Cn;
+        dim3 grid(nbig + small_rows * Cs), block(kGemmThreads);
+#define PK2_GEMM_RBANDS(TB, X)                                                                                                  \
+  hipLaunchKernelGGL((gemm_f32_rows_bands_kernel<TB, X>), grid, block, 0, stream, M, N, K, alpha, A, lda, B, ldb, beta, C, ldc, \
+                     bias, vecA, vecB, nbig, Cn, m_split, Cs, rmap)
+        if (transb) { if (x3) PK2_GEMM_RBANDS(true, true); else PK2_GEMM_RBANDS(true, false); }
+        else        { if (x3) PK2_GEMM_RBANDS(false, true); else PK2_GEMM_RBANDS(false, false); }
+#undef PK2_GEMM_RBANDS
+        PK2_LAUNCH_CHECK();
+        return PK2_OK;
+      }
+      if (map != kMapNone) {
+        launch(best_r > 0 ? 2 : 1, 0, M);
+        PK2_LAUNCH_CHECK();
+        return PK2_OK;
+      }
       if (best_r > 0 && one_launch) {
         const int m_split = best_r * 128, small_rows = (M - m_split + 63) / 64;
         const int nbig = best_r * Cn;
@@ -372,6 +526,58 @@
   return pk2_colsum_f32(A, lda, K, M, 1.0f, colsum, stream_);
 }
 
+extern "C" int pk2_gemm_f32_rows(int32_t transb, int32_t M_total, int32_t N, int32_t K, float alpha, const float* A, int64_t lda,
+                                 const float* B, int64_t ldb, float beta, float* C, int64_t ldc, const float* bias,
+                                 const int32_t* rmap, int32_t Mv, void* stream_) {
+  if (!rmap || Mv == M_total) return pk2_gemm_f32(0, transb, M_total, N, K, alpha, A, lda, B, ldb, beta, C, ldc, bias, stream_);
+  PK2_REQUIRE(A && B && C && N > 0 && K > 0 && Mv > 0 && Mv < M_total, "gemm_f32_rows: bad args");
+  GemmBatch bt{1, 0, 0, 0, 0, 0, 0, 1, 0};
+  return gemm_launch(0, transb, Mv, N, K, alpha, A, lda, B, ldb, beta, C, ldc, bias, 1, bt, true, static_cast<hipStream_t>(stream_),
+                     rmap, kMapRows);
+}
+
+extern "C" int pk2_gemm_f32_tn_colsum_rows(int32_t M, int32_t N, int32_t K_total, float alpha, const float* A, int64_t lda,
+                                           const float* B, int64_t ldb, float beta, float* C, int64_t ldc, float* colsum,
+                                           const int32_t* rmap, int32_t Kv, void* stream_) {
+  if (!rmap || Kv == K_total) return pk2_gemm_f32_tn_colsum(M, N, K_total, alpha, A, lda, B, ldb, beta, C, ldc, colsum, stream_);
+  PK2_REQUIRE(A && B && C && colsum && M > 0 && N > 0 && Kv > 0 && Kv < K_total, "gemm_f32_tn_colsum_rows: bad args");
+  GemmBatch bt{1, 0, 0, 0, 0, 0, 0, 1, 0};
+  const bool fuse = gemm_arith() == 1;
+  if (fuse) bt.colsum = colsum;
+  hipStream_t stream = static_cast<hipStream_t>(stream_);
+  int rc = gemm_launch(1, 0, M, N, Kv, alpha, A, lda, B, ldb, beta, C, ldc, nullptr, 1, bt, true, stream, rmap, kMapK);
+  if (rc || fuse) return rc;
+  const int col_blocks = (M + 63) / 64;
+  const int splits = std::max(1, std::min((Kv + 63) / 64, 1024 / col_blocks));
+  const int rows_per_block = (Kv + splits - 1) / splits;
+  hipLaunchKernelGGL(colsum_rows_kernel, dim3(col_blocks, (Kv + rows_per_block - 1) / rows_per_block), dim3(256), 0, stream, A, lda, Kv,
+                     M, rows_per_block, colsum, rmap);
+  PK2_LAUNCH_CHECK();
+  return PK2_OK;
+}
+
+extern "C" int pk2_rows_zero(float* X, int64_t ldx, int32_t N, const int32_t* rows, int32_t n, void* stream_) {
+  PK2_REQUIRE(X && rows && N > 0 && n >= 0 && ldx >= N, "rows_zero: bad args");
+  if (n == 0) return PK2_OK;
+  const bool vec = (N & 3) == 0 && (ldx & 3) == 0 && (reinterpret_cast<uintptr_t>(X) & 15) == 0;
+  const int per = vec ? 1024 : 256;
+  hipLaunchKernelGGL((rows_zero_or_pack_kernel<false>), dim3(std::min((N + per - 1) / per, 64), std::min(n, 4096)), dim3(256), 0,
+                     static_cast<hipStream_t>(stream_), X, ldx, N, rows, n, (float*)nullptr, (int64_t)0, vec);
+  PK2_LAUNCH_CHECK();
+  return PK2_OK;
+}
+
+extern "C" int pk2_rows_pack(const float* X, int64_t ldx, int32_t N, const int32_t* rows, int32_t n, float* out, int64_t ldo,
+                             void* stream_) {
+  PK2_REQUIRE(X && rows && out && N > 0 && n > 0 && ldx >= N && ldo >= N, "rows_pack: bad args");
+  const bool vec = (N & 3) == 0 && (ldx & 3) == 0 && (ldo & 3) == 0 && ((reinterpret_cast<uintptr_t>(X) | reinterpret_cast<uintptr_t>(out)) & 15) == 0;
+  const int per = vec ? 1024 : 256;
+  hipLaunchKernelGGL((rows_zero_or_pack_kernel<true>), dim3(std::min((N + per - 1) / per, 64), std::min(n, 4096)), dim3(256), 0,
+                     static_cast<hipStream_t>(stream_), const_cast<float*>(X), ldx, N, rows, n, out, ldo, vec);
+  PK2_LAUNCH_CHECK();
+  return PK2_OK;
+}
+
 extern "C" int pk2_gemm_f32_batched(int32_t transa, int32_t transb, int32_t M, int32_t N, int32_t K, float alpha,
                                     const float* A, int64_t lda, int64_t strideA0, int64_t strideA1,
                                     const float* B, int64_t ldb, int64_t strideB0, int64_t strideB1, float beta,
diff --git a/pykaldi2_amd/csrc/gemm_tile.h b/pykaldi2_amd/csrc/gemm_tile.h
--- a/pykaldi2_amd/csrc/gemm_tile.h
+++ b/pykaldi2_amd/csrc/gemm_tile.h
@@ -19,9 +19,11 @@
   template <bool KCONTIG> static constexpr int ld() { return KCONTIG ? LDK : LD; }
 };
 
-template <bool KCONTIG, int TILES>
+constexpr int kMapNone = 0, kMapRows = 1, kMapK = 2;
+template <bool KCONTIG, int TILES, int MAP = kMapNone>
 __device__ __forceinline__ void load_slab(const float* __restrict__ base, int64_t ld, int r0, int k0,
-                                          int R, int K, bool vec, float4 (&reg)[TILES]) {
+                                          int R, int K, bool vec, float4 (&reg)[TILES], const int* __restrict__ rmap = nullptr) {
+  static_assert(MAP == kMapNone || (MAP == kMapRows && KCONTIG) || (MAP == kMapK && !KCONTIG), "which operand layout a map applies to");
   const int tid = threadIdx.x;
 #pragma unroll
   for (int h = 0; h < TILES; ++h) {
@@ -30,6 +32,31 @@
     else         { k = tid / Geo<TILES>::LPK + h * (kGemmThreads / Geo<TILES>::LPK); r = (tid % Geo<TILES>::LPK) * 4; }
     const int gr = r0 + r, gk = k0 + k;
     float4 v = make_float4(0.f, 0.f, 0.f, 0.f);
+    if constexpr (MAP == kMapRows) {
+      if (gr < R) {
+        const float* p = base + (int64_t)rmap[gr] * ld + gk;
+        if (vec && gk + 3 < K) {
+          v = *reinterpret_cast<const float4*>(p);
+        } else {
+          if (gk + 0 < K) v.x = p[0];
+          if (gk + 1 < K) v.y = p[1];
+          if (gk + 2 < K) v.z = p[2];
+          if (gk + 3 < K) v.w = p[3];
+        }
+      }
+    } else if constexpr (MAP == kMapK) {
+      if (gk < K) {
+        const float* p = base + (int64_t)rmap[gk] * ld + gr;
+        if (vec && gr + 3 < R) {
+          v = *reinterpret_cast<const float4*>(p);
+        } else {
+          if (gr + 0 < R) v.x = p[0];
+          if (gr + 1 < R) v.y = p[1];
+          if (gr + 2 < R) v.z = p[2];
+          if (gr + 3 < R) v.w = p[3];
+        }
+      }
+    } else
     if (KCONTIG) {
       if (gr < R) {
         const float* p = base + (int64_t)gr * ld + gk;
@@ -60,14 +87,16 @@
 }
 
 
-template <bool KCONTIG, int TILES>
+template <bool KCONTIG, int TILES, bool ROWMAP = false>
 __device__ __forceinline__ void slab_pointers(const float* __restrict__ base, int64_t ld, int r0, int k0, int R,
-                                              const float* (&ptr)[TILES], int64_t* step) {
+                                              const float* (&ptr)[TILES], int64_t* step, const int* __restrict__ rmap = nullptr) {
   const int tid = threadIdx.x;
 #pragma unroll
   for (int h = 0; h < TILES; ++h) {
     if (KCONTIG) {
       const int r = (tid >> 2) + h * 64, k = (tid & 3) * 4;
+      if constexpr (ROWMAP) ptr[h] = base + (int64_t)rmap[min(r0 + r, R - 1)] * ld + k0 + k;
+      else
       ptr[h] = base + (int64_t)min(r0 + r, R - 1) * ld + k0 + k;
     } else {
       const int k = tid / Geo<TILES>::LPK + h * (kGemmThreads / Geo<TILES>::LPK), r = (tid % Geo<TILES>::LPK) * 4;
@@ -109,12 +138,14 @@
   }
 }
 
-template <bool KCA, bool KCB, int TILES>
+template <bool KCA, bool KCB, int TILES, int MAP = kMapNone>
 __device__ __forceinline__ void tile_mainloop(const float* __restrict__ A, int64_t lda, const float* __restrict__ B, int64_t ldb,
                                               int m0, int n0, int kbeg, int K, int M, int N, bool vecA, bool vecB,
                                               float (*As)[BK * Geo<TILES>::template ld<KCA>()],
                                               float (*Bs)[BK * Geo<TILES>::template ld<KCB>()],
-                                              f32x16 (&acc)[TILES][TILES], bool zero_acc = true) {
+                                              f32x16 (&acc)[TILES][TILES], bool zero_acc = true, const int* __restrict__ rmap = nullptr) {
+  static_assert(MAP == kMapNone || (MAP == kMapRows && KCA) || (MAP == kMapK && !KCA && !KCB), "kMapRows: rows of a k-contiguous A; kMapK: both operands row-contiguous");
+  constexpr int MAPA = MAP, MAPB = MAP == kMapK ? kMapK : kMapNone;
   constexpr int BM = Geo<TILES>::BMN, BN = Geo<TILES>::BMN;
   constexpr int LDA = Geo<TILES>::template ld<KCA>(), LDB = Geo<TILES>::template ld<KCB>();
   const int lane = threadIdx.x & 63, w = threadIdx.x >> 6;
@@ -142,8 +173,22 @@
                         (n0 + BN <= N || KCB || ((N & 3) == 0 && N >= 4));
   const float* pa[TILES]; const float* pb[TILES];
   int64_t stepA = 0, stepB = 0;
+  if constexpr (MAP == kMapK) {
+    slab_pointers<KCA, TILES>(A, lda, m0, 0, M, pa, &stepA);
+    slab_pointers<KCB, TILES>(B, ldb, n0, 0, N, pb, &stepB);
+#pragma unroll
+    for (int h = 0; h < TILES; ++h) {
+      const int k = threadIdx.x / Geo<TILES>::LPK + h * (kGemmThreads / Geo<TILES>::LPK);
+      pa[h] -= (int64_t)k * lda;
+      pb[h] -= (int64_t)k * ldb;
+    }
+  } else if constexpr (MAP == kMapRows) {
+    slab_pointers<KCA, TILES, true>(A, lda, m0, kbeg, M, pa, &stepA, rmap);
+    slab_pointers<KCB, TILES>(B, ldb, n0, kbeg, N, pb, &stepB);
+  } else {
   slab_pointers<KCA, TILES>(A, lda, m0, kbeg, M, pa, &stepA);
   slab_pointers<KCB, TILES>(B, ldb, n0, kbeg, N, pb, &stepB);
+  }
 #ifndef PK2_GEMM_HOIST
 #define PK2_GEMM_HOIST 8
 #endif
@@ -204,13 +249,35 @@
   };
   if (interior) {
     const int nk_fast = (K - kbeg) / BK;
+    if constexpr (MAP == kMapK) {
+      int mk[TILES];
+#pragma unroll
+      for (int h = 0; h < TILES; ++h) mk[h] = nk_fast > 0 ? rmap[kbeg + threadIdx.x / Geo<TILES>::LPK + h * (kGemmThreads / Geo<TILES>::LPK)] : 0;
+      pipeline(nk_fast, [&](int ks, float4 (&xa)[TILES], float4 (&xb)[TILES]) {
+        int nm[TILES];
+        const int kn = kbeg + min(ks + 1, nk_fast - 1) * BK + threadIdx.x / Geo<TILES>::LPK;
+#pragma unroll
+        for (int h = 0; h < TILES; ++h) nm[h] = rmap[kn + h * (kGemmThreads / Geo<TILES>::LPK)];
+#pragma unroll
+        for (int h = 0; h < TILES; ++h) xa[h] = *reinterpret_cast<const float4*>(pa[h] + (int64_t)mk[h] * lda);
+#pragma unroll
+        for (int h = 0; h < TILES; ++h) xb[h] = *reinterpret_cast<const float4*>(pb[h] + (int64_t)mk[h] * ldb);
+#pragma unroll
+        for (int h = 0; h < TILES; ++h) mk[h] = nm[h];
+      });
+    } else
     pipeline(nk_fast, [&](int ks, float4 (&xa)[TILES], float4 (&xb)[TILES]) {
       load_slab_fast<TILES>(pa, ks * stepA, xa);
       load_slab_fast<TILES>(pb, ks * stepB, xb);
     });
     if (nk > nk_fast) {
+      if constexpr (MAP != kMapNone) {
+        load_slab<KCA, TILES, MAPA>(A, lda, m0, kbeg + nk_fast * BK, M, K, vecA, ra[0], rmap);
+        load_slab<KCB, TILES, MAPB>(B, ldb, n0, kbeg + nk_fast * BK, N, K, vecB, rb[0], rmap);
+      } else {
       load_slab<KCA, TILES>(A, lda, m0, kbeg + nk_fast * BK, M, K, vecA, ra[0]);
       load_slab<KCB, TILES>(B, ldb, n0, kbeg + nk_fast * BK, N, K, vecB, rb[0]);
+      }
       store_slab<KCA, TILES>(As[0], ra[0]);
       store_slab<KCB, TILES>(Bs[0], rb[0]);
       lds_barrier();
@@ -218,6 +285,12 @@
       lds_barrier();
     }
   } else {
+    if constexpr (MAP != kMapNone)
+      pipeline(nk, [&](int ks, float4 (&xa)[TILES], float4 (&xb)[TILES]) {
+        load_slab<KCA, TILES, MAPA>(A, lda, m0, kbeg + ks * BK, M, K, vecA, xa, rmap);
+        load_slab<KCB, TILES, MAPB>(B, ldb, n0, kbeg + ks * BK, N, K, vecB, xb, rmap);
+      });
+    else
     pipeline(nk, [&](int ks, float4 (&xa)[TILES], float4 (&xb)[TILES]) {
       load_slab<KCA, TILES>(A, lda, m0, kbeg + ks * BK, M, K, vecA, xa);
       load_slab<KCB, TILES>(B, ldb, n0, kbeg + ks * BK, N, K, vecB, xb);
diff --git a/pykaldi2_amd/fbank.py b/pykaldi2_amd/fbank.py
--- a/pykaldi2_amd/fbank.py
+++ b/pykaldi2_amd/fbank.py
@@ -68,6 +68,12 @@
 
     @staticmethod
     def pad_roll_subsample(feats, row_off, frames, shift=0, subsample=1, time_major=False):
+        x = FbankExtractor._pad_roll_subsample(feats, row_off, frames, shift, subsample, time_major)
+        x.pk2_lengths = row_lengths(frames, shift, subsample)
+        return x
+
+    @staticmethod
+    def _pad_roll_subsample(feats, row_off, frames, shift, subsample, time_major):
         n = len(frames)
         max_t = int(max(frames))
         out_t = (max_t - 1) // subsample + 1
@@ -77,6 +83,11 @@
                                                      int(subsample), _lib.ptr(x), out_t, 1 if time_major else 0,
                                                      _lib.stream_ptr(feats.device)))
         return x
+
+
+def row_lengths(frames, shift=0, subsample=1):
+    out_t = (int(max(frames)) - 1) // subsample + 1
+    return tuple(min(out_t, -(-(int(f) + max(int(shift), 0)) // subsample)) for f in frames)
 
 
 def utt2seg(feats, seg_len, seg_shift):
diff --git a/pykaldi2_amd/lstm.py b/pykaldi2_amd/lstm.py
--- a/pykaldi2_amd/lstm.py
+++ b/pykaldi2_amd/lstm.py
@@ -50,10 +50,40 @@
         nn.init.uniform_(self.bias, -bound, bound)
 
 
+_row_map_cache = {}
+
+
+def row_map_host(lengths, T, B):
+    import numpy as np
+    lens = np.asarray(lengths, dtype=np.int64)
+    if lens.shape != (B,) or (lens < 0).any() or (lens > T).any():
+        raise ValueError("lengths: one frame count in [0, T] per sequence (B = %d, T = %d): %r" % (B, T, list(lengths)))
+    valid = (np.arange(T)[:, None] < lens[None, :]).reshape(-1)
+    return np.concatenate([np.flatnonzero(valid), np.flatnonzero(~valid)]).astype(np.int32), int(valid.sum())
+
+
+def _row_map(lengths, T, B, dev):
+    key = (tuple(int(v) for v in lengths), T, B)
+    hit = _row_map_cache.get(key)
+    if hit is None:
+        if len(_row_map_cache) >= 4096:
+            _row_map_cache.clear()
+        perm, mv = row_map_host(key[0], T, B)
+        hit = _row_map_cache[key] = (torch.from_numpy(perm).pin_memory(), mv)
+    host, mv = hit
+    if mv == T * B or mv == 0:
+        return None
+    return host.to(dev, non_blocking=True), mv
+
+
+def _p32(t, off_ints=0):
+    return ctypes.c_void_p(t.data_ptr() + 4 * off_ints)
+
+
 class _LstmAmFunction(torch.autograd.Function):
 
     @staticmethod
-    def forward(ctx, x_tm, model, *params):
+    def forward(ctx, x_tm, model, lengths, *params):
         m = model
         T, B, Din = x_tm.shape
         H, D, Lr = m.hidden_size, m.num_dirs, m.num_layers
@@ -93,8 +123,16 @@
                 seeds.append(None)
         P = m.output_size
         logits = torch.empty(T, B, P, device=dev, dtype=torch.float32)
-        _gemm(0, 1, rows, P, D * H, _p(inp), D * H, _p(m.output_layer.weight), D * H, _p(logits), P,
-              bias=_p(m.output_layer.bias))
+        rm = _row_map(lengths, T, B, dev) if lengths is not None and os.environ.get("PK2_OUT_ROWS", "1") != "0" else None
+        if rm is not None:
+            rmap, mv = rm
+            _lib.check(L.pk2_gemm_f32_rows(1, rows, P, D * H, 1.0, _p(inp), D * H, _p(m.output_layer.weight), D * H, 0.0,
+                                           _p(logits), P, _p(m.output_layer.bias), _p32(rmap), mv, sp))
+            _lib.check(L.pk2_rows_zero(_p(logits), P, P, _p32(rmap, mv), rows - mv, sp))
+        else:
+            _gemm(0, 1, rows, P, D * H, _p(inp), D * H, _p(m.output_layer.weight), D * H, _p(logits), P,
+                  bias=_p(m.output_layer.bias))
+        ctx.row_map = rm
         ctx.model = m
         ctx.saved = saved
         ctx.seeds = seeds
@@ -130,11 +168,29 @@
 
         gw, gb = views["output_layer.weight"], views["output_layer.bias"]
         dy = torch.empty(T, B, D * H, device=dev, dtype=torch.float32)
-        _gemm(0, 0, rows, D * H, P, _p(dlogits), P, _p(m.output_layer.weight), D * H, _p(dy), D * H)
+        rm = ctx.row_map
+        if rm is not None:
+            rmap, mv = rm
+            _lib.check(L.pk2_gemm_f32_rows(0, rows, D * H, P, 1.0, _p(dlogits), P, _p(m.output_layer.weight), D * H, 0.0,
+                                           _p(dy), D * H, None, _p32(rmap), mv, sp))
+            _lib.check(L.pk2_rows_zero(_p(dy), D * H, D * H, _p32(rmap, mv), rows - mv, sp))
+        else:
+            _gemm(0, 0, rows, D * H, P, _p(dlogits), P, _p(m.output_layer.weight), D * H, _p(dy), D * H)
 
         def out_grads():
-            _lib.check(L.pk2_gemm_f32_tn_colsum(P, D * H, rows, 1.0, _p(dlogits), P, _p(y_last), D * H, 1.0, _p(gw), D * H, _p(gb),
-                                                _lib.stream_ptr()))
+            if rm is not None and os.environ.get("PK2_OUT_ROWS_WGRAD", "map") == "pack":
+                dl_p = torch.empty(mv, P, device=dev, dtype=torch.float32)
+                y_p = torch.empty(mv, D * H, device=dev, dtype=torch.float32)
+                _lib.check(L.pk2_rows_pack(_p(dlogits), P, P, _p32(rmap), mv, _p(dl_p), P, _lib.stream_ptr()))
+                _lib.check(L.pk2_rows_pack(_p(y_last), D * H, D * H, _p32(rmap), mv, _p(y_p), D * H, _lib.stream_ptr()))
+                _lib.check(L.pk2_gemm_f32_tn_colsum(P, D * H, mv, 1.0, _p(dl_p), P, _p(y_p), D * H, 1.0, _p(gw), D * H, _p(gb),
+                                                    _lib.stream_ptr()))
+            elif rm is not None:
+                _lib.check(L.pk2_gemm_f32_tn_colsum_rows(P, D * H, rows, 1.0, _p(dlogits), P, _p(y_last), D * H, 1.0, _p(gw),
+                                                         D * H, _p(gb), _p32(rmap), mv, _lib.stream_ptr()))
+            else:
+                _lib.check(L.pk2_gemm_f32_tn_colsum(P, D * H, rows, 1.0, _p(dlogits), P, _p(y_last), D * H, 1.0, _p(gw), D * H,
+                                                    _p(gb), _lib.stream_ptr()))
             m._bucket_ready("output_layer")
         on_side(out_grads, dlogits, y_last)
         scratch = torch.empty(L.pk2_lstm_bwd_scratch_floats(B, H, D), device=dev, dtype=torch.float32)
@@ -196,7 +252,7 @@
             if p.grad is None or p.grad.data_ptr() != v.data_ptr():
                 p.grad = v
         ctx.saved = None
-        return (dx, None) + (None,) * len(m._param_names)
+        return (dx, None, None) + (None,) * len(m._param_names)
 
 
 class LSTMAM(nn.Module):
@@ -300,7 +356,13 @@
             lo, hi = self._buckets[name]
             self._bucket_hook(name, self._gflat[lo:hi])
 
-    def forward_time_major(self, x_tm):
+    def forward_time_major(self, x_tm, lengths=None):
+        if lengths is None:
+            lengths = getattr(x_tm, "pk2_lengths", None)
+        if lengths is not None:
+            lengths = tuple(int(v) for v in lengths)
+            if len(lengths) != x_tm.shape[1] or min(lengths) < 0 or max(lengths) > x_tm.shape[0]:
+                raise ValueError("lengths: one frame count in [0, T] per sequence, got %r for x_tm %r" % (lengths, tuple(x_tm.shape)))
         _lib.require_gpu()
         assert x_tm.is_cuda and x_tm.dtype == torch.float32
         self._ensure_flat()
@@ -309,7 +371,7 @@
             in_size = self.input_size if l == 0 else H * D
             assert (4 * H * in_size) % 64 == 0 and (4 * H * H) % 64 == 0 and (4 * H) % 64 == 0
         params = [p for _, p in self.named_parameters()]
-        return _LstmAmFunction.apply(x_tm, self, *params)
+        return _LstmAmFunction.apply(x_tm, self, lengths, *params)
 
     def forward(self, data):
         x_tm = data.transpose(0, 1).contiguous()
```

Result: faster. 4895 (median of 6 runs) (+1.3%).
